# jamesli1618/Obj-GAN

Measured on AMD Instinct MI355X. Metric: G+D train-step images/sec at 256x256, batch 16 per GPU, higher is better.
Workload: dtype fp32 (fp16x2: operands as two fp16 pieces of x * 2^s on the fp16 MFMA); 1 GPU; stage3_256x256_full_GD_step: RNN_ENCODER+G_NET(3 stages)+PatD x3+ShpD x3+ObjSSD+ObjLSD(ROIAlign)+DAMSM+KL+Adam x9+EMA+IS-monitor; per_gpu_batch=16, global_batch=16, parallelism=dp1, fresh_batch_every_step=True

## Files before the change

### include/objgan_hip.h

```cpp
#ifndef OBJGAN_HIP_H
#define OBJGAN_HIP_H

#ifdef __cplusplus
extern "C" {
#endif

int objgan_roi_align_forward(const float* features, const float* rois, float* output,
                             int num_rois, int roi_cols, int channels, int height, int width,
                             int aligned_height, int aligned_width, float spatial_scale,
                             void* stream);
int objgan_roi_align_backward(const float* top_grad, const float* rois, float* bottom_grad,
                              int batch_size, int num_rois, int roi_cols, int channels,
                              int height, int width, int aligned_height, int aligned_width,
                              float spatial_scale, void* stream);

long objgan_roi_align_backward_ws_floats(int batch_size, int num_rois, int channels, int height, int width,
                                         int aligned_height, int aligned_width);
int objgan_roi_align_backward_ordered(const float* top_grad, const float* rois, float* bottom_grad,
                                      int batch_size, int num_rois, int roi_cols, int channels,
                                      int height, int width, int aligned_height, int aligned_width,
                                      float spatial_scale, float* ws, long ws_floats, void* stream);
int objgan_avgpool2s1_forward(const float* in, float* out, long planes, int ih, int iw, void* stream);
int objgan_avgpool2s1_backward(const float* grad_out, float* grad_in, long planes, int ih, int iw,
                               void* stream);

long objgan_conv_packed_floats(int M, int C, int T);
int objgan_conv_bank_layout(int N, int C, int H, int W, int M, int Tg, int PH, int PW, int act, int math);
int objgan_conv_igemm(const float* x, const float* w, const float* bias, float* y, float* wt,
                      int N, int C, int H, int W, int upsample, int pad_mode,
                      int Cout, int Cin, int Torig, int transpose,
                      int Tg, const int* dh, const int* dw, const int* src_tap,
                      int PH, int PW, int stride,
                      int OHf, int OWf, int osh, int osw, int ooh, int oow,
                      int act, int y_prezeroed, int wt_packed, int math, float* ring, const float* xmax, float* ymax,
                      float* ws, long ws_floats, void* stream);
int objgan_absmax_partials(const float* x, long n, float* out1024, void* stream);
long objgan_h2_records_floats(int N, int C, long HW);
int objgan_h2_records(const float* x, const float* xmax1024, void* rec, int N, int C, long HW, void* stream);
long objgan_conv_igemm_ws_floats(int N, int C, int H, int W, int upsample, int pad_mode,
                                 int Cout, int Cin, int Torig, int transpose, int Tg,
                                 int PH, int PW, int stride, int OHf, int OWf, int osh, int osw,
                                 int act, int y_prezeroed, int math, int ring);
int objgan_conv_igemm_plan(int N, int C, int H, int W, int upsample, int pad_mode,
                           int Cout, int Cin, int Torig, int transpose, int Tg,
                           int PH, int PW, int stride, int OHf, int OWf, int osh, int osw,
                           int act, int y_prezeroed, int math, int ring, int* out);
int objgan_reflect_ring_fold(const float* ring, float* y, long planes, int H, int W, void* stream);
long objgan_conv_dgrad_s2_phases_ws_floats(int N, int Cout, int OH, int OW, int math);
int objgan_conv_dgrad_s2_phases_plan(int N, int Cout, int OH, int OW, int Cin, int Tg, int PH, int PW, int math, int* out);
long objgan_conv_dgrad_s2_thin_floats(int Cout, int Cin);
int objgan_conv_pack_job_thin_phase(void* job, const float* w, float* wt, int Cout, int Cin, int phase);
int objgan_conv_dgrad_s2_thin(const float* dy, const float* w, float* dx, float* wt, int N, int Cout, int OH, int OW,
                              int Cin, int wt_packed, void* stream);
int objgan_conv_dgrad_s2_phases(const float* x, const float* w, float* y, float* wt,
                                int N, int Cout, int OH, int OW, int Cin, int Torig,
                                int Tg, const int* dh, const int* dw, const int* src_tap,
                                int PH, int PW, int wt_packed, int math, const float* xmax, float* ws, long ws_floats,
                                void* stream);
long objgan_conv_wgrad_ws_floats(int N, int Cin, int H, int W, int upsample, int pad_mode,
                                 int Cout, int OH, int OW, int ksize, int stride, int pad, int math);
int objgan_conv_wgrad_plan(int N, int Cin, int H, int W, int upsample, int pad_mode,
                           int Cout, int OH, int OW, int ksize, int stride, int pad, int math, int* out);
int objgan_conv_wgrad(const float* x, const float* dy, float* dw,
                      int N, int Cin, int H, int W, int upsample, int pad_mode,
                      int Cout, int OH, int OW, int ksize, int stride, int pad, int math,
                      int accumulate, const float* xmax, const float* dymax, float* ws, long ws_floats, void* stream);
int objgan_conv_wgrad_rec_ok(int N, int Cin, int H, int W, int Cout, int OH, int OW, int ksize);
long objgan_nhwc_bf16_floats(int N, int C, long HW);
int objgan_nhwc_bf16(const float* x, float* out, int N, int C, long HW, void* stream);
int objgan_conv_wgrad_bfb_ok(int N, int Cin, int H, int W, int Cout, int OH, int OW, int ksize);

int objgan_lstm_bidir_forward(const float* table, const long* captions, const int* lens,
                              const float* wt_ih, const float* wt_hh, const float* b_ih, const float* b_hh,
                              float* out, float* hn, int B, int L, int Lout, int I, int H, int ntoken,
                              void* stream);
int objgan_lstm_bidir_forward_state(const float* table, const long* captions, const int* lens,
                                    const float* wt_ih, const float* wt_hh, const float* b_ih, const float* b_hh,
                                    float* out, float* hn, float* cn, int B, int L, int Lout, int I, int H,
                                    int ntoken, void* stream);

int objgan_box_decode_default_cpw(void);
int objgan_box_decode(const float* h0, const float* c0, const double* noise,
                      const float* l_emb, const float* xy_w, const float* xy_b, const float* wh_w, const float* wh_b,
                      const float* nxy_w, const float* nxy_b, const float* wt_ih, const float* wt_hh,
                      const float* b_ih, const float* b_hh, const float* lo_wt, const float* lo_b,
                      const float* xyo_wt, const float* xyo_b, const float* who_wt, const float* who_b,
                      float x0, float y0, float w0, float r0,
                      int* labels, int* lengths, double* samples, float* trace,
                      int B, int T, int H, int L, int K, int A, int sos, int eos, int cpw, void* stream);

long objgan_box_train_ws_floats(int B, int T, int H, int L, int K, int A);
int objgan_box_train_forward(const float* h0, const float* c0, const int* labels, const float* boxes, const int* lens,
                             const float* l_emb, const float* xy_w, const float* xy_b, const float* wh_w,
                             const float* wh_b, const float* nxy_w, const float* nxy_b, const float* wt_ih,
                             const float* wt_hh, const float* b_ih, const float* b_hh, const float* lo_wt,
                             const float* lo_b, const float* xyo_wt, const float* xyo_b, const float* who_wt,
                             const float* who_b, float x0, float y0, float w0, float r0, float* trace, float* ws,
                             long ws_floats, int B, int T, int H, int L, int K, int A, int cpw, void* stream);
int objgan_box_train_loss(const float* trace, const int* labels, const float* boxes, const int* lens,
                          const float* weight, float lamda1, float lamda2, double* sums, float* dtrace,
                          int B, int T, int L, int K, int pad, void* stream);
int objgan_box_train_backward(const float* dtrace, const float* trace, const float* c0, const int* labels,
                              const int* lens, const float* wt_ih, const float* wt_hh, const float* lo_wt,
                              const float* xyo_wt, const float* who_wt, float* const* grads, float* ws, long ws_floats,
                              int B, int T, int H, int L, int K, int A, int cpw, void* stream);
int objgan_box_train_clip(const float* g, long n, float max_norm, double* partials, float* out, void* stream);

long objgan_norm_ws_floats(int N, int C, int HW, int per_channel);
int objgan_norm_forward(const float* x, float* y, const float* residual,
                        const float* gamma, const float* beta,
                        float* running_mean, float* running_var,
                        float* sums, float* mean, float* rstd,
                        int N, int C, int HW, int per_channel, int mode,
                        float eps, float momentum, float* amax, void* stream);
int objgan_norm_amax_supported(int N, int C, int HW, int per_channel, int affine);
int objgan_norm_apply(const float* x, float* y, const float* residual, const float* gamma, const float* beta,
                      const float* mean, const float* rstd, int N, int C, int HW, int per_channel, int mode,
                      void* stream);
int objgan_norm_backward(const float* x, const float* dy, const float* mean, const float* rstd,
                         const float* gamma, const float* beta, float* bsums,
                         float* dx, float* dgamma, float* dbeta,
                         int N, int C, int HW, int per_channel, int mode, float* amax, void* stream);
int objgan_act_backward(const float* dy, const float* y, float* dz, long total, int kind, float* amax, void* stream);
long objgan_channel_sum_ws_floats(int N, int C, int HW);
int objgan_channel_sum(const float* x, float* out, int N, int C, int HW, float* ws, void* stream);

int objgan_attn_general_forward(const float* x, const float* src, const unsigned char* mask,
                                float* wc, float* attn, int B, int idf, int Q, int L, void* stream);
long objgan_attn_general_backward_ws_floats(int B, int idf, int Q, int L);
int objgan_attn_general_backward(const float* x, const float* src, const float* attn,
                                 const float* dwc, const float* dattn, float* dx, float* dsrc,
                                 int B, int idf, int Q, int L, float* ws, void* stream);
int objgan_attn_bu_forward(const float* tgt, const float* ctx1, const float* src,
                           const unsigned char* mask, float* wc, float* attn,
                           int B, int d2, int idf, int R, int L, int normalize, float eps,
                           void* stream);
int objgan_attn_bu_backward(const float* dwc, const float* attn, float* dsrc,
                            int B, int idf, int R, int L, void* stream);
int objgan_masked_max_forward(const float* f, const float* m, float* out, int B, int num, int R,
                              int P, long m_stride_b, long m_stride_r, long m_stride_c, void* stream);
long objgan_masked_max_backward_ws_floats(int B, int num, int R, int P);
int objgan_masked_max_backward(const float* f, const float* m, const float* dout, float* df,
                               int B, int num, int R, int P, long m_stride_b, long m_stride_r,
                               long m_stride_c, float* ws, void* stream);
int objgan_softmax_strided_forward(const float* x, float* y, long outer, int dim, long inner,
                                   float scale, const int* lens, int nlens,
                                   const unsigned char* rowvalid, void* stream);
int objgan_softmax_strided_backward(const float* y, const float* dy, float* dx, long outer, int dim,
                                    long inner, float scale, void* stream);

int objgan_bilinear_forward(const float* x, float* y, long planes, int ih, int iw, int oh, int ow,
                            void* stream);
int objgan_bilinear_backward(const float* dy, float* dx, long planes, int ih, int iw, int oh, int ow,
                             void* stream);
int objgan_sum2x2(const float* dy, float* dx, long planes, int h, int w, void* stream);
int objgan_reflect_fold(const float* dxp, float* dx, long planes, int h, int w, void* stream);
int objgan_bce_const_forward(const float* p, float* out, int n, float t, void* stream);
int objgan_bce_const_backward(const float* p, const float* g, float* dp, int n, float t, void* stream);
int objgan_conv_pack_job_bytes();
int objgan_conv_pack_job(void* job, const float* w, float* wt, int N, int C, int H, int W, int Cout, int Cin,
                         int Torig, int transpose, int Tg, const int* src_tap, int PH, int PW, int act, int math);
int objgan_conv_pack_job_phase(void* job, const float* w, float* wt, int Cout, int Cin, int Torig, int Tg,
                               const int* src_tap_phase, int phase, int math);
int objgan_conv_pack_jobs_run(const void* jobs_dev, int njobs, void* stream);
int objgan_bmm_strided(const float* A, const float* B, float* C, int batch, int M, int N, int K,
                       long sab, long sam, long sak, long sbb, long sbk, long sbn,
                       long scb, long scm, long scn, void* stream);
int objgan_lift_taps_forward(const float* z, const float* bias, float* y, float* scratch, int N, int Mo, int h,
                             int w, int SH, int SW, const int* ci0, const int* ci1, const float* cl1,
                             const int* ri0, const int* ri1, const float* rl1, void* stream);
int objgan_lift_taps_backward(const float* dy, float* dz, float* scratch, int N, int Mo, int h, int w, int SH,
                              int SW, const int* roff, const int* ridx, const float* rwt, const int* coff,
                              const int* cidx, const float* cwt, void* stream);
int objgan_pool2d_forward(const float* x, float* y, int* idx, long planes, int H, int W, int OH, int OW,
                          int k, int s, int p, int mode, void* stream);
int objgan_pool2d_backward(const float* dy, const int* idx, float* dx, long planes, int H, int W, int OH,
                           int OW, int k, int s, int p, int mode, void* stream);
int objgan_adam_step(float* p, const float* g, float* m, float* v, long n, double lr, double beta1,
                     double beta2, double eps, int step, float grad_scale, void* stream);
int objgan_adam_step_gated(float* p, const float* g, float* m, float* v, long n, double lr, double beta1,
                           double beta2, double eps, double* state, const float* flag, float* coef,
                           float grad_scale, void* stream);
int objgan_ema_update(float* avg, const float* p, long n, float decay, float one_minus_decay,
                      void* stream);

int objgan_resize_pil_kmax(int max_in, int S);
int objgan_resize_pil_rgb8(const unsigned char* src, const long* offs, const int* hs, const int* ws, int B,
                           int Hmax, int kmax, int S, int* coef_scratch, unsigned char* tmp_scratch, float* out,
                           void* stream);

long objgan_jpeg_desc_bytes(void);
long objgan_jpeg_seg_bytes(void);
int objgan_jpeg_parse(const unsigned char* file, long nbytes, void* desc_out);
long objgan_jpeg_plan(void* descs, int n, const long* file_offsets, const long* out_offsets, const int* nsegs);
int objgan_jpeg_decode(const unsigned char* files, const void* descs_host, const void* descs_dev, int n,
                       unsigned char* out, void* ws, long ws_bytes, const void* index_in, void* index_out, void* stream);

int objgan_mask_resize(const double* src, int count, int n, int nsizes, const int* sizes, double* const* out,
                       const int* ntaps, const double* taps, void* stream);

int objgan_bilinear_halfpixel_forward(const float* x, float* y, int N, int C, int H, int W, int OH, int OW,
                                      const float* scale, const float* shift, void* stream);
int objgan_moments_accumulate(const float* x, int rows, int D, double* sum, double* outer, void* stream);
int objgan_moments_finalize(const double* sum, const double* outer, long n, int D, double* mu, double* sigma,
                            void* stream);

long objgan_snapshot_ws_doubles(int nvis, int T, int a, int vis);
int objgan_snapshot_blend_table(unsigned char* table65536);
int objgan_snapshot_grid(const float* imgs, const float* lr_imgs, const float* attn, const int* counts, const double* M,
                         const unsigned char* strip, unsigned char* out, double* ws, long ws_doubles,
                         int nvis, int T, int a, int vis, int H, int W, int LH, int LW,
                         int max_word_num, int font_max, int per_panel_norm, void* stream);
int objgan_mask_to_rgb8(const float* masks, const int* sel, unsigned char* out, int N, int HW, void* stream);

int objgan_convlstm_cell_forward(const float* gx, const float* gh, const float* c_prev, float* h_out, float* h_slab,
                                 float* c_out, float* acts, int B, int Ch, int HW, long gx_bstride, long slab_bstride,
                                 void* stream);
int objgan_convlstm_cell_backward(const float* dh_slab, const float* dh_rec, const float* dc_in, const float* acts,
                                  const float* c_prev, float* dg_slab, float* dg_out, float* dc_out, int B, int Ch, int HW,
                                  long dh_bstride, long dg_bstride, void* stream);
int objgan_box_max_forward(const float* x, float* y, unsigned char* arg, int B, int R, long CSS, void* stream);
int objgan_box_max_backward(const float* dy, const unsigned char* arg, float* dx, int B, int R, long CSS, void* stream);
int objgan_boxmaps_onehot(const float* raw, const int* cat, const int* num, float* fwd, float* bwd, int B, int NB, int R,
                          int C, int SS, void* stream);

int objgan_layout_from_decode(const int* labels, const int* lengths, const double* samples, const double* mean_std,
                              const int* label_to_cat, const int* cat_to_rel, const int* thresholds,
                              double* boxes, int* nbox, double* rois, double* fm_rois, int* num_rois, int* cats,
                              float* maps, float* fmaps, int* bounds, const int* sizes, int NB, int F, int R,
                              int min_size, int tie_rule, int B, int T, int L, int ncat, void* stream);

int objgan_pcp_stem_forward(const float* x, float* y, int N, int S, int OH, int OW, void* stream);
int objgan_pcp_stem_backward(const float* dy, float* dx, int N, int S, int OH, int OW, void* stream);
long objgan_l1_tap_ws_doubles(long n);
int objgan_l1_tap_forward(const float* f, const float* r, long n, float* out, int slot, double* ws, void* stream);
int objgan_l1_tap_backward(const float* f, const float* r, const float* gdown, const float* coef, float* g, long n,
                           int relu_mask, float* amax, void* stream);

int objgan_prof_enable(int on);
int objgan_prof_collect(double* ms, double* flops, long* count);
int objgan_prof_dump(float* ms, double* flops, int* meta, int max_records, int* n_out);

#ifdef __cplusplus
}
#endif
#endif
```

### obj-gan_amd/csrc/norm.hip

```cpp
#include "common.h"

#define OG_NORM_NONE 0
#define OG_NORM_LRELU 1
#define OG_NORM_GLU 2

struct NormGeom {
    int N, C, HW;
    int per_channel;
};

__device__ __forceinline__ float og_sigmoid(float v) { return 1.0f / (1.0f + expf(-v)); }

struct NormWs { float* sums; float* part; int P; };
__device__ __forceinline__ void og_store_partial2(const NormWs& ws, int g, int idx, float s1, float s2) {
    if (ws.P == 1) { ws.sums[2 * g] = s1; ws.sums[2 * g + 1] = s2; return; }
    float* slot = ws.part + ((size_t)g * ws.P + idx) * 2;
    slot[0] = s1; slot[1] = s2;
}
__global__ __launch_bounds__(256) void norm_partials_sum_kernel(NormWs ws, int G, float* __restrict__ amax) {
    if (amax && blockIdx.x == 0)
        for (int k = threadIdx.x; k < OG_AMAX_SLOTS; k += 256) amax[k] = 0.f;
    const int g = blockIdx.x * blockDim.x + threadIdx.x;
    if (g >= G) return;
    const float* p = ws.part + (size_t)g * ws.P * 2;
    float a = 0.f, b = 0.f;
    for (int k = 0; k < ws.P; ++k) { a += p[2 * k]; b += p[2 * k + 1]; }
    ws.sums[2 * g] = a; ws.sums[2 * g + 1] = b;
}

__global__ __launch_bounds__(256) void norm_stats_kernel(const float* __restrict__ x,
                                                         NormWs ws, NormGeom gm) {
    __shared__ float red[16];
    const int g = blockIdx.x;
    const int planes = gm.per_channel ? gm.N : 1;
    const size_t base = gm.per_channel ? (size_t)g * gm.HW : (size_t)g * gm.HW;
    const size_t pstride = (size_t)gm.C * gm.HW;
    const long total = (long)planes * gm.HW;
    const float K = x[base];
    const long chunk = (total + gridDim.y - 1) / gridDim.y;
    const long e0 = (long)blockIdx.y * chunk;
    const long e1 = min(total, e0 + chunk);
    float s1 = 0.f, s2 = 0.f;
    for (long e = e0 + threadIdx.x; e < e1; e += blockDim.x) {
        const long p = e / gm.HW;
        const long i = e - p * gm.HW;
        const float d = x[base + p * pstride + i] - K;
        s1 += d;
        s2 += d * d;
    }
    s1 = og_block_sum(s1, red);
    s2 = og_block_sum(s2, red);
    if (threadIdx.x == 0) og_store_partial2(ws, g, blockIdx.y, s1, s2);
}

__global__ __launch_bounds__(256) void norm_finalize_kernel(
    const float* __restrict__ x, const float* __restrict__ sums, float* __restrict__ mean,
    float* __restrict__ rstd, float* __restrict__ running_mean, float* __restrict__ running_var,
    NormGeom gm, int G, float eps, float momentum) {
    const int g = blockIdx.x * blockDim.x + threadIdx.x;
    if (g >= G) return;
    const float cnt = gm.per_channel ? (float)gm.N * gm.HW : (float)gm.HW;
    const float K = x[(size_t)g * gm.HW];
    const float m1 = sums[2 * g] / cnt;
    float var = sums[2 * g + 1] / cnt - m1 * m1;
    var = fmaxf(var, 0.f);
    const float mu = K + m1;
    mean[g] = mu;
    rstd[g] = 1.0f / sqrtf(var + eps);
    if (running_mean) {
        const float unbiased = cnt > 1.f ? var * cnt / (cnt - 1.f) : var;
        running_mean[g] = (1.f - momentum) * running_mean[g] + momentum * mu;
        running_var[g] = (1.f - momentum) * running_var[g] + momentum * unbiased;
    }
}

__global__ __launch_bounds__(256) void norm_apply_kernel(
    const float* __restrict__ x, const float* __restrict__ mean, const float* __restrict__ rstd,
    const float* __restrict__ gamma, const float* __restrict__ beta,
    const float* __restrict__ residual, float* __restrict__ y, NormGeom gm, int mode) {
    const int Co = mode == OG_NORM_GLU ? gm.C / 2 : gm.C;
    const long total = (long)gm.N * Co * gm.HW;
    for (long e = (long)blockIdx.x * blockDim.x + threadIdx.x; e < total;
         e += (long)gridDim.x * blockDim.x) {
        const long plane = e / gm.HW;
        const int i = (int)(e - plane * gm.HW);
        const int n = (int)(plane / Co);
        const int c = (int)(plane - (long)n * Co);
        const int ga = gm.per_channel ? c : n * gm.C + c;
        const size_t xa = ((size_t)n * gm.C + c) * gm.HW + i;
        float za = (x[xa] - mean[ga]) * rstd[ga];
        if (gamma) za = za * gamma[c] + beta[c];
        float v;
        if (mode == OG_NORM_GLU) {
            const int cb = c + Co;
            const int gb = gm.per_channel ? cb : n * gm.C + cb;
            float zb = (x[xa + (size_t)Co * gm.HW] - mean[gb]) * rstd[gb];
            if (gamma) zb = zb * gamma[cb] + beta[cb];
            v = za * og_sigmoid(zb);
        } else if (mode == OG_NORM_LRELU) {
            v = za > 0.f ? za : 0.2f * za;
        } else {
            v = za;
        }
        if (residual) v += residual[e];
        y[e] = v;
    }
}

__device__ __forceinline__ float norm_dz(const float* __restrict__ x, const float* __restrict__ dy,
                                         const float* __restrict__ mean, const float* __restrict__ rstd,
                                         const float* __restrict__ gamma, const float* __restrict__ beta,
                                         const NormGeom& gm, int mode, int n, int c, int i,
                                         float& xhat_out) {
    const int g = gm.per_channel ? c : n * gm.C + c;
    const size_t xa = ((size_t)n * gm.C + c) * gm.HW + i;
    const float xhat = (x[xa] - mean[g]) * rstd[g];
    xhat_out = xhat;
    if (mode == OG_NORM_NONE) return dy[xa];
    float z = xhat;
    if (gamma) z = z * gamma[c] + beta[c];
    if (mode == OG_NORM_LRELU) return dy[xa] * (z > 0.f ? 1.f : 0.2f);
    const int Ch = gm.C / 2;
    const bool is_gate = c >= Ch;
    const int co = is_gate ? c - Ch : c;
    const int cp = is_gate ? c - Ch : c + Ch;
    const int gp = gm.per_channel ? cp : n * gm.C + cp;
    const size_t xp = ((size_t)n * gm.C + cp) * gm.HW + i;
    float zp = (x[xp] - mean[gp]) * rstd[gp];
    if (gamma) zp = zp * gamma[cp] + beta[cp];
    const float d = dy[((size_t)n * Ch + co) * gm.HW + i];
    if (!is_gate) return d * og_sigmoid(zp);
    const float sg = og_sigmoid(z);
    return d * zp * sg * (1.f - sg);
}

__global__ __launch_bounds__(256) void norm_bwd_stats_kernel(
    const float* __restrict__ x, const float* __restrict__ dy, const float* __restrict__ mean,
    const float* __restrict__ rstd, const float* __restrict__ gamma, const float* __restrict__ beta,
    NormWs ws, NormGeom gm, int mode) {
    __shared__ float red[16];
    const int g = blockIdx.x;
    const int planes = gm.per_channel ? gm.N : 1;
    const long total = (long)planes * gm.HW;
    const long chunk = (total + gridDim.y - 1) / gridDim.y;
    const long e0 = (long)blockIdx.y * chunk;
    const long e1 = min(total, e0 + chunk);
    float s1 = 0.f, s2 = 0.f;
    for (long e = e0 + threadIdx.x; e < e1; e += blockDim.x) {
        const int p = (int)(e / gm.HW);
        const int i = (int)(e - (long)p * gm.HW);
        const int n = gm.per_channel ? p : g / gm.C;
        const int c = gm.per_channel ? g : g - n * gm.C;
        float xhat;
        const float dz = norm_dz(x, dy, mean, rstd, gamma, beta, gm, mode, n, c, i, xhat);
        s1 += dz;
        s2 += dz * xhat;
    }
    s1 = og_block_sum(s1, red);
    s2 = og_block_sum(s2, red);
    if (threadIdx.x == 0) og_store_partial2(ws, g, blockIdx.y, s1, s2);
}

__global__ __launch_bounds__(256) void norm_bwd_apply_kernel(
    const float* __restrict__ x, const float* __restrict__ dy, const float* __restrict__ mean,
    const float* __restrict__ rstd, const float* __restrict__ gamma, const float* __restrict__ beta,
    const float* __restrict__ bsums, float* __restrict__ dx, NormGeom gm, int mode) {
    const long total = (long)gm.N * gm.C * gm.HW;
    const float inv_cnt = 1.0f / (gm.per_channel ? (float)gm.N * gm.HW : (float)gm.HW);
    for (long e = (long)blockIdx.x * blockDim.x + threadIdx.x; e < total;
         e += (long)gridDim.x * blockDim.x) {
        const long plane = e / gm.HW;
        const int i = (int)(e - plane * gm.HW);
        const int n = (int)(plane / gm.C);
        const int c = (int)(plane - (long)n * gm.C);
        const int g = gm.per_channel ? c : n * gm.C + c;
        float xhat;
        const float dz = norm_dz(x, dy, mean, rstd, gamma, beta, gm, mode, n, c, i, xhat);
        const float gw = gamma ? gamma[c] : 1.f;
        dx[e] = gw * rstd[g] * (dz - bsums[2 * g] * inv_cnt - xhat * bsums[2 * g + 1] * inv_cnt);
    }
}

#define OG_NORM_CHUNK 8192

__device__ __forceinline__ float og_group_mean(const float* p, int g) { return p[g]; }

__global__ __launch_bounds__(256) void norm_stats_plane_kernel(const float* __restrict__ x,
                                                               NormWs ws, NormGeom gm) {
    __shared__ float red[16];
    const int plane = blockIdx.x;
    const int c = plane % gm.C;
    const int g = gm.per_channel ? c : plane;
    const float K = x[(size_t)g * gm.HW];
    const float4* xp = reinterpret_cast<const float4*>(x + (size_t)plane * gm.HW);
    const int i0 = blockIdx.y * (OG_NORM_CHUNK / 4);
    const int i1 = min(gm.HW / 4, i0 + OG_NORM_CHUNK / 4);
    float s1 = 0.f, s2 = 0.f;
    for (int i = i0 + threadIdx.x; i < i1; i += 256) {
        const float4 v = xp[i];
        const float a = v.x - K, b = v.y - K, cc = v.z - K, d = v.w - K;
        s1 += (a + b) + (cc + d);
        s2 += (a * a + b * b) + (cc * cc + d * d);
    }
    s1 = og_block_sum(s1, red);
    s2 = og_block_sum(s2, red);
    const int idx = gm.per_channel ? (plane / gm.C) * (int)gridDim.y + (int)blockIdx.y : (int)blockIdx.y;
    if (threadIdx.x == 0) og_store_partial2(ws, g, idx, s1, s2);
}

struct NormFin { const float* sums; float* mean_out; float* rstd_out; float* running_mean; float* running_var;
                 float eps, momentum; };

__device__ __forceinline__ void og_group_stats(const float* __restrict__ x, const NormFin& fin, const NormGeom& gm,
                                               int g, bool publish, float& mu, float& rs) {
    const float cnt = gm.per_channel ? (float)gm.N * gm.HW : (float)gm.HW;
    const float K = x[(size_t)g * gm.HW];
    const float m1 = fin.sums[2 * g] / cnt;
    float var = fin.sums[2 * g + 1] / cnt - m1 * m1;
    var = fmaxf(var, 0.f);
    mu = K + m1;
    rs = 1.0f / sqrtf(var + fin.eps);
    if (publish && threadIdx.x == 0) {
        fin.mean_out[g] = mu;
        fin.rstd_out[g] = rs;
        if (fin.running_mean) {
            const float unbiased = cnt > 1.f ? var * cnt / (cnt - 1.f) : var;
            fin.running_mean[g] = (1.f - fin.momentum) * fin.running_mean[g] + fin.momentum * mu;
            fin.running_var[g] = (1.f - fin.momentum) * fin.running_var[g] + fin.momentum * unbiased;
        }
    }
}

template <int MODE>
__global__ __launch_bounds__(256) void norm_apply_plane_kernel(
    const float* __restrict__ x, const float* __restrict__ mean, const float* __restrict__ rstd,
    const float* __restrict__ gamma, const float* __restrict__ beta,
    const float* __restrict__ residual, float* __restrict__ y, NormGeom gm, NormFin fin, float* __restrict__ amax) {
    __shared__ float amax_red[4];
    float vmax = 0.f;
    const int Co = MODE == OG_NORM_GLU ? gm.C / 2 : gm.C;
    const int plane = blockIdx.x;
    const int n = plane / Co;
    const int c = plane - n * Co;
    const int ga = gm.per_channel ? c : n * gm.C + c;
    const bool publish = blockIdx.y == 0 && (!gm.per_channel || n == 0);
    float mua, rsa;
    if (fin.sums) og_group_stats(x, fin, gm, ga, publish, mua, rsa); else { mua = mean[ga]; rsa = rstd[ga]; }
    float sa = rsa, ta = -mua * sa;
    if (gamma) { ta = ta * gamma[c] + beta[c]; sa *= gamma[c]; }
    float sb = 0.f, tb = 0.f;
    if (MODE == OG_NORM_GLU) {
        const int cb = c + Co;
        const int gb = gm.per_channel ? cb : n * gm.C + cb;
        float mub, rsb;
        if (fin.sums) og_group_stats(x, fin, gm, gb, publish, mub, rsb); else { mub = mean[gb]; rsb = rstd[gb]; }
        sb = rsb; tb = -mub * sb;
        if (gamma) { tb = tb * gamma[cb] + beta[cb]; sb *= gamma[cb]; }
    }
    const float4* xa = reinterpret_cast<const float4*>(x + ((size_t)n * gm.C + c) * gm.HW);
    const float4* xb = reinterpret_cast<const float4*>(x + ((size_t)n * gm.C + c + Co) * gm.HW);
    const float4* rp = residual ? reinterpret_cast<const float4*>(residual + (size_t)plane * gm.HW) : nullptr;
    float4* yp = reinterpret_cast<float4*>(y + (size_t)plane * gm.HW);
    const int i0 = blockIdx.y * (OG_NORM_CHUNK / 4);
    const int i1 = min(gm.HW / 4, i0 + OG_NORM_CHUNK / 4);
    for (int i = i0 + threadIdx.x; i < i1; i += 256) {
        const float4 a = xa[i];
        float z[4] = {a.x * sa + ta, a.y * sa + ta, a.z * sa + ta, a.w * sa + ta};
        float v[4];
        if (MODE == OG_NORM_GLU) {
            const float4 b = xb[i];
            const float zb[4] = {b.x * sb + tb, b.y * sb + tb, b.z * sb + tb, b.w * sb + tb};
#pragma unroll
            for (int j = 0; j < 4; ++j) v[j] = z[j] * og_sigmoid(zb[j]);
        } else if (MODE == OG_NORM_LRELU) {
#pragma unroll
            for (int j = 0; j < 4; ++j) v[j] = z[j] > 0.f ? z[j] : 0.2f * z[j];
        } else {
#pragma unroll
            for (int j = 0; j < 4; ++j) v[j] = z[j];
        }
        if (rp) { const float4 r = rp[i]; v[0] += r.x; v[1] += r.y; v[2] += r.z; v[3] += r.w; }
        yp[i] = make_float4(v[0], v[1], v[2], v[3]);
        vmax = fmaxf(fmaxf(vmax, fmaxf(fabsf(v[0]), fabsf(v[1]))), fmaxf(fabsf(v[2]), fabsf(v[3])));
    }
    if (amax) og_amax_atomic(og_block_max(vmax, amax_red), amax, blockIdx.x + blockIdx.y * gridDim.x);
}

template <int MODE>
__device__ __forceinline__ void norm_dz_pair(float xa, float xb, float d, float ma, float ra, float mb, float rb,
                                             float gaa, float baa, float gab, float bab, bool affine,
                                             float& dza, float& xha, float& dzb, float& xhb) {
    xha = (xa - ma) * ra;
    float za = affine ? xha * gaa + baa : xha;
    if (MODE == OG_NORM_NONE) { dza = d; dzb = 0.f; xhb = 0.f; return; }
    if (MODE == OG_NORM_LRELU) { dza = d * (za > 0.f ? 1.f : 0.2f); dzb = 0.f; xhb = 0.f; return; }
    xhb = (xb - mb) * rb;
    const float zb = affine ? xhb * gab + bab : xhb;
    const float sg = og_sigmoid(zb);
    dza = d * sg;
    dzb = d * za * sg * (1.f - sg);
}

template <int MODE>
__global__ __launch_bounds__(256) void norm_bwd_stats_plane_kernel(
    const float* __restrict__ x, const float* __restrict__ dy, const float* __restrict__ mean,
    const float* __restrict__ rstd, const float* __restrict__ gamma, const float* __restrict__ beta,
    NormWs ws, NormGeom gm) {
    __shared__ float red[16];
    const int Co = MODE == OG_NORM_GLU ? gm.C / 2 : gm.C;
    const int plane = blockIdx.x;
    const int n = plane / Co;
    const int c = plane - n * Co;
    const int cb = c + Co;
    const int ga = gm.per_channel ? c : n * gm.C + c;
    const int gb = gm.per_channel ? cb : n * gm.C + cb;
    const bool affine = gamma != nullptr;
    const float ma = mean[ga], ra = rstd[ga];
    const float mb = MODE == OG_NORM_GLU ? mean[gb] : 0.f, rb = MODE == OG_NORM_GLU ? rstd[gb] : 0.f;
    const float gaa = affine ? gamma[c] : 1.f, baa = affine ? beta[c] : 0.f;
    const float gab = (affine && MODE == OG_NORM_GLU) ? gamma[cb] : 1.f, bab = (affine && MODE == OG_NORM_GLU) ? beta[cb] : 0.f;
    const float4* xa = reinterpret_cast<const float4*>(x + ((size_t)n * gm.C + c) * gm.HW);
    const float4* xb = reinterpret_cast<const float4*>(x + ((size_t)n * gm.C + cb) * gm.HW);
    const float4* dp = reinterpret_cast<const float4*>(dy + (size_t)plane * gm.HW);
    const int i0 = blockIdx.y * (OG_NORM_CHUNK / 4);
    const int i1 = min(gm.HW / 4, i0 + OG_NORM_CHUNK / 4);
    float a1 = 0.f, a2 = 0.f, b1 = 0.f, b2 = 0.f;
    for (int i = i0 + threadIdx.x; i < i1; i += 256) {
        const float4 va = xa[i];
        const float4 vb = MODE == OG_NORM_GLU ? xb[i] : make_float4(0.f, 0.f, 0.f, 0.f);
        const float4 vd = dp[i];
        const float xs[4] = {va.x, va.y, va.z, va.w}, ys[4] = {vb.x, vb.y, vb.z, vb.w}, ds[4] = {vd.x, vd.y, vd.z, vd.w};
#pragma unroll
        for (int j = 0; j < 4; ++j) {
            float dza, xha, dzb, xhb;
            norm_dz_pair<MODE>(xs[j], ys[j], ds[j], ma, ra, mb, rb, gaa, baa, gab, bab, affine, dza, xha, dzb, xhb);
            a1 += dza; a2 += dza * xha;
            if (MODE == OG_NORM_GLU) { b1 += dzb; b2 += dzb * xhb; }
        }
    }
    a1 = og_block_sum(a1, red);
    a2 = og_block_sum(a2, red);
    if (MODE == OG_NORM_GLU) { b1 = og_block_sum(b1, red); b2 = og_block_sum(b2, red); }
    const int idx = gm.per_channel ? n * (int)gridDim.y + (int)blockIdx.y : (int)blockIdx.y;
    if (threadIdx.x == 0) {
        og_store_partial2(ws, ga, idx, a1, a2);
        if (MODE == OG_NORM_GLU) og_store_partial2(ws, gb, idx, b1, b2);
    }
}

template <int MODE>
__global__ __launch_bounds__(256) void norm_bwd_apply_plane_kernel(
    const float* __restrict__ x, const float* __restrict__ dy, const float* __restrict__ mean,
    const float* __restrict__ rstd, const float* __restrict__ gamma, const float* __restrict__ beta,
    const float* __restrict__ bsums, float* __restrict__ dx, NormGeom gm,
    float* __restrict__ dgamma, float* __restrict__ dbeta, float* __restrict__ amax) {
    __shared__ float amax_red[4];
    float vmax = 0.f;
    const int Co = MODE == OG_NORM_GLU ? gm.C / 2 : gm.C;
    const int plane = blockIdx.x;
    const int n = plane / Co;
    const int c = plane - n * Co;
    const int cb = c + Co;
    const int ga = gm.per_channel ? c : n * gm.C + c;
    const int gb = gm.per_channel ? cb : n * gm.C + cb;
    const bool affine = gamma != nullptr;
    const float inv_cnt = 1.0f / (gm.per_channel ? (float)gm.N * gm.HW : (float)gm.HW);
    if (dgamma && gm.per_channel && n == 0 && blockIdx.y == 0 && threadIdx.x == 0) {
        dbeta[c] = bsums[2 * c]; dgamma[c] = bsums[2 * c + 1];
        if (MODE == OG_NORM_GLU) { dbeta[cb] = bsums[2 * cb]; dgamma[cb] = bsums[2 * cb + 1]; }
    }
    const float ma = mean[ga], ra = rstd[ga];
    const float mb = MODE == OG_NORM_GLU ? mean[gb] : 0.f, rb = MODE == OG_NORM_GLU ? rstd[gb] : 0.f;
    const float gaa = affine ? gamma[c] : 1.f, baa = affine ? beta[c] : 0.f;
    const float gab = (affine && MODE == OG_NORM_GLU) ? gamma[cb] : 1.f, bab = (affine && MODE == OG_NORM_GLU) ? beta[cb] : 0.f;
    const float ka1 = bsums[2 * ga] * inv_cnt, ka2 = bsums[2 * ga + 1] * inv_cnt;
    const float kb1 = MODE == OG_NORM_GLU ? bsums[2 * gb] * inv_cnt : 0.f, kb2 = MODE == OG_NORM_GLU ? bsums[2 * gb + 1] * inv_cnt : 0.f;
    const float wa = gaa * ra, wb = gab * rb;
    const float4* xa = reinterpret_cast<const float4*>(x + ((size_t)n * gm.C + c) * gm.HW);
    const float4* xb = reinterpret_cast<const float4*>(x + ((size_t)n * gm.C + cb) * gm.HW);
    const float4* dp = reinterpret_cast<const float4*>(dy + (size_t)plane * gm.HW);
    float4* oa = reinterpret_cast<float4*>(dx + ((size_t)n * gm.C + c) * gm.HW);
    float4* ob = reinterpret_cast<float4*>(dx + ((size_t)n * gm.C + cb) * gm.HW);
    const int i0 = blockIdx.y * (OG_NORM_CHUNK / 4);
    const int i1 = min(gm.HW / 4, i0 + OG_NORM_CHUNK / 4);
    for (int i = i0 + threadIdx.x; i < i1; i += 256) {
        const float4 va = xa[i];
        const float4 vb = MODE == OG_NORM_GLU ? xb[i] : make_float4(0.f, 0.f, 0.f, 0.f);
        const float4 vd = dp[i];
        const float xs[4] = {va.x, va.y, va.z, va.w}, ys[4] = {vb.x, vb.y, vb.z, vb.w}, ds[4] = {vd.x, vd.y, vd.z, vd.w};
        float ra4[4], rb4[4];
#pragma unroll
        for (int j = 0; j < 4; ++j) {
            float dza, xha, dzb, xhb;
            norm_dz_pair<MODE>(xs[j], ys[j], ds[j], ma, ra, mb, rb, gaa, baa, gab, bab, affine, dza, xha, dzb, xhb);
            ra4[j] = wa * (dza - ka1 - xha * ka2);
            rb4[j] = wb * (dzb - kb1 - xhb * kb2);
        }
        oa[i] = make_float4(ra4[0], ra4[1], ra4[2], ra4[3]);
        if (MODE == OG_NORM_GLU) ob[i] = make_float4(rb4[0], rb4[1], rb4[2], rb4[3]);
#pragma unroll
        for (int j = 0; j < 4; ++j) vmax = fmaxf(vmax, fmaxf(fabsf(ra4[j]), MODE == OG_NORM_GLU ? fabsf(rb4[j]) : 0.f));
    }
    if (amax) og_amax_atomic(og_block_max(vmax, amax_red), amax, blockIdx.x + blockIdx.y * gridDim.x);
}


__device__ __forceinline__ void og_block_sum2(float& a, float& b, float* red) {
    a = og_wave_sum(a);
    b = og_wave_sum(b);
    const int lane = threadIdx.x & 63, wid = threadIdx.x >> 6;
    __syncthreads();
    if (lane == 0) { red[wid] = a; red[4 + wid] = b; }
    __syncthreads();
    a = red[0] + red[1] + red[2] + red[3];
    b = red[4] + red[5] + red[6] + red[7];
}

template <int MODE>
__global__ __launch_bounds__(256) void in_fwd_fused_kernel(
    const float* __restrict__ x, const float* __restrict__ residual, float* __restrict__ y,
    float* __restrict__ mean, float* __restrict__ rstd, NormGeom gm, float eps, float* __restrict__ amax) {
    __shared__ float red[8];
    float vmax = 0.f;
    const int Co = MODE == OG_NORM_GLU ? gm.C / 2 : gm.C;
    const int plane = blockIdx.x;
    const int n = plane / Co;
    const int c = plane - n * Co;
    const int ga = n * gm.C + c, gb = ga + Co;
    const float4* xa = reinterpret_cast<const float4*>(x + (size_t)ga * gm.HW);
    const float4* xb = reinterpret_cast<const float4*>(x + (size_t)gb * gm.HW);
    const int n4 = gm.HW / 4;
    const float inv = 1.0f / (float)gm.HW;
    const float Ka = x[(size_t)ga * gm.HW];
    float s1 = 0.f, s2 = 0.f;
    for (int i = threadIdx.x; i < n4; i += 256) {
        const float4 v = xa[i];
        const float a = v.x - Ka, b = v.y - Ka, cc = v.z - Ka, d = v.w - Ka;
        s1 += (a + b) + (cc + d);
        s2 += (a * a + b * b) + (cc * cc + d * d);
    }
    og_block_sum2(s1, s2, red);
    float m1 = s1 * inv;
    float var = fmaxf(s2 * inv - m1 * m1, 0.f);
    const float mua = Ka + m1, ra = 1.0f / sqrtf(var + eps);
    float mub = 0.f, rb = 0.f;
    if (MODE == OG_NORM_GLU) {
        const float Kb = x[(size_t)gb * gm.HW];
        s1 = 0.f; s2 = 0.f;
        for (int i = threadIdx.x; i < n4; i += 256) {
            const float4 v = xb[i];
            const float a = v.x - Kb, b = v.y - Kb, cc = v.z - Kb, d = v.w - Kb;
            s1 += (a + b) + (cc + d);
            s2 += (a * a + b * b) + (cc * cc + d * d);
        }
        og_block_sum2(s1, s2, red);
        m1 = s1 * inv;
        var = fmaxf(s2 * inv - m1 * m1, 0.f);
        mub = Kb + m1; rb = 1.0f / sqrtf(var + eps);
    }
    if (threadIdx.x == 0) {
        mean[ga] = mua; rstd[ga] = ra;
        if (MODE == OG_NORM_GLU) { mean[gb] = mub; rstd[gb] = rb; }
    }
    const float sa = ra, ta = -mua * ra, sb = rb, tb = -mub * rb;
    const float4* rp = residual ? reinterpret_cast<const float4*>(residual + (size_t)plane * gm.HW) : nullptr;
    float4* yp = reinterpret_cast<float4*>(y + (size_t)plane * gm.HW);
    for (int i = threadIdx.x; i < n4; i += 256) {
        const float4 a = xa[i];
        const float z[4] = {a.x * sa + ta, a.y * sa + ta, a.z * sa + ta, a.w * sa + ta};
        float v[4];
        if (MODE == OG_NORM_GLU) {
            const float4 b = xb[i];
            const float zb[4] = {b.x * sb + tb, b.y * sb + tb, b.z * sb + tb, b.w * sb + tb};
#pragma unroll
            for (int j = 0; j < 4; ++j) v[j] = z[j] * og_sigmoid(zb[j]);
        } else if (MODE == OG_NORM_LRELU) {
#pragma unroll
            for (int j = 0; j < 4; ++j) v[j] = z[j] > 0.f ? z[j] : 0.2f * z[j];
        } else {
#pragma unroll
            for (int j = 0; j < 4; ++j) v[j] = z[j];
        }
        if (rp) { const float4 r = rp[i]; v[0] += r.x; v[1] += r.y; v[2] += r.z; v[3] += r.w; }
        yp[i] = make_float4(v[0], v[1], v[2], v[3]);
        vmax = fmaxf(fmaxf(vmax, fmaxf(fabsf(v[0]), fabsf(v[1]))), fmaxf(fabsf(v[2]), fabsf(v[3])));
    }
    if (amax) og_amax_atomic(og_block_max(vmax, red), amax, blockIdx.x);
}

template <int MODE>
__global__ __launch_bounds__(256) void in_bwd_fused_kernel(
    const float* __restrict__ x, const float* __restrict__ dy, const float* __restrict__ mean,
    const float* __restrict__ rstd, float* __restrict__ dx, NormGeom gm, float* __restrict__ amax) {
    __shared__ float red[8];
    float vmax = 0.f;
    const int Co = MODE == OG_NORM_GLU ? gm.C / 2 : gm.C;
    const int plane = blockIdx.x;
    const int n = plane / Co;
    const int c = plane - n * Co;
    const int ga = n * gm.C + c, gb = ga + Co;
    const float inv_cnt = 1.0f / (float)gm.HW;
    const float ma = mean[ga], ra = rstd[ga];
    const float mb = MODE == OG_NORM_GLU ? mean[gb] : 0.f, rb = MODE == OG_NORM_GLU ? rstd[gb] : 0.f;
    const float4* xa = reinterpret_cast<const float4*>(x + (size_t)ga * gm.HW);
    const float4* xb = reinterpret_cast<const float4*>(x + (size_t)gb * gm.HW);
    const float4* dp = reinterpret_cast<const float4*>(dy + (size_t)plane * gm.HW);
    float4* oa = reinterpret_cast<float4*>(dx + (size_t)ga * gm.HW);
    float4* ob = reinterpret_cast<float4*>(dx + (size_t)gb * gm.HW);
    const int n4 = gm.HW / 4;
    float a1 = 0.f, a2 = 0.f, b1 = 0.f, b2 = 0.f;
    for (int i = threadIdx.x; i < n4; i += 256) {
        const float4 va = xa[i];
        const float4 vb = MODE == OG_NORM_GLU ? xb[i] : make_float4(0.f, 0.f, 0.f, 0.f);
        const float4 vd = dp[i];
        const float xs[4] = {va.x, va.y, va.z, va.w}, ys[4] = {vb.x, vb.y, vb.z, vb.w}, ds[4] = {vd.x, vd.y, vd.z, vd.w};
#pragma unroll
        for (int j = 0; j < 4; ++j) {
            float dza, xha, dzb, xhb;
            norm_dz_pair<MODE>(xs[j], ys[j], ds[j], ma, ra, mb, rb, 1.f, 0.f, 1.f, 0.f, false, dza, xha, dzb, xhb);
            a1 += dza; a2 += dza * xha;
            if (MODE == OG_NORM_GLU) { b1 += dzb; b2 += dzb * xhb; }
        }
    }
    og_block_sum2(a1, a2, red);
    if (MODE == OG_NORM_GLU) og_block_sum2(b1, b2, red);
    const float ka1 = a1 * inv_cnt, ka2 = a2 * inv_cnt, kb1 = b1 * inv_cnt, kb2 = b2 * inv_cnt;
    for (int i = threadIdx.x; i < n4; i += 256) {
        const float4 va = xa[i];
        const float4 vb = MODE == OG_NORM_GLU ? xb[i] : make_float4(0.f, 0.f, 0.f, 0.f);
        const float4 vd = dp[i];
        const float xs[4] = {va.x, va.y, va.z, va.w}, ys[4] = {vb.x, vb.y, vb.z, vb.w}, ds[4] = {vd.x, vd.y, vd.z, vd.w};
        float ra4[4], rb4[4];
#pragma unroll
        for (int j = 0; j < 4; ++j) {
            float dza, xha, dzb, xhb;
            norm_dz_pair<MODE>(xs[j], ys[j], ds[j], ma, ra, mb, rb, 1.f, 0.f, 1.f, 0.f, false, dza, xha, dzb, xhb);
            ra4[j] = ra * (dza - ka1 - xha * ka2);
            rb4[j] = rb * (dzb - kb1 - xhb * kb2);
        }
        oa[i] = make_float4(ra4[0], ra4[1], ra4[2], ra4[3]);
        if (MODE == OG_NORM_GLU) ob[i] = make_float4(rb4[0], rb4[1], rb4[2], rb4[3]);
#pragma unroll
        for (int j = 0; j < 4; ++j) vmax = fmaxf(vmax, fmaxf(fabsf(ra4[j]), MODE == OG_NORM_GLU ? fabsf(rb4[j]) : 0.f));
    }
    if (amax) og_amax_atomic(og_block_max(vmax, red), amax, blockIdx.x);
}

__global__ void norm_affine_grad_kernel(const float* __restrict__ bsums, float* __restrict__ dgamma,
                                        float* __restrict__ dbeta, int C) {
    const int c = blockIdx.x * blockDim.x + threadIdx.x;
    if (c < C) { dbeta[c] = bsums[2 * c]; dgamma[c] = bsums[2 * c + 1]; }
}

__device__ __forceinline__ float act_bwd_one(float d, float o, int kind) {
    float r;
    if (kind == 1) r = d * (o > 0.f ? 1.f : 0.2f);
    else if (kind == 2) r = d * (1.f - o * o);
    else if (kind == 3) r = d * o * (1.f - o);
    else r = o > 0.f ? d : 0.f;
    return r;
}
template <bool V4>
__global__ __launch_bounds__(256) void act_bwd_kernel(const float* __restrict__ dy,
                                                      const float* __restrict__ y,
                                                      float* __restrict__ dz, long total, int kind,
                                                      float* __restrict__ amax) {
    __shared__ float amax_red[4];
    float vmax = 0.f;
    long e0 = 0;
    if (V4) {
        const long n4 = total >> 2, step = (long)gridDim.x * 256;
        const float4* d4 = reinterpret_cast<const float4*>(dy);
        const float4* y4 = reinterpret_cast<const float4*>(y);
        float4* z4 = reinterpret_cast<float4*>(dz);
        for (long g = (long)blockIdx.x * 256 + threadIdx.x; g < n4; g += 2 * step) {
            const long g1 = g + step < n4 ? g + step : g;
            const float4 da = d4[g], oa = y4[g], db = d4[g1], ob = y4[g1];
            const float ra[4] = {act_bwd_one(da.x, oa.x, kind), act_bwd_one(da.y, oa.y, kind),
                                 act_bwd_one(da.z, oa.z, kind), act_bwd_one(da.w, oa.w, kind)};
            const float rb[4] = {act_bwd_one(db.x, ob.x, kind), act_bwd_one(db.y, ob.y, kind),
                                 act_bwd_one(db.z, ob.z, kind), act_bwd_one(db.w, ob.w, kind)};
            z4[g] = make_float4(ra[0], ra[1], ra[2], ra[3]);
            if (g1 != g) z4[g1] = make_float4(rb[0], rb[1], rb[2], rb[3]);
#pragma unroll
            for (int j = 0; j < 4; ++j) vmax = fmaxf(vmax, fmaxf(fabsf(ra[j]), fabsf(rb[j])));
        }
        e0 = n4 << 2;
    }
    for (long e = e0 + (long)blockIdx.x * blockDim.x + threadIdx.x; e < total;
         e += (long)gridDim.x * blockDim.x) {
        const float r = act_bwd_one(dy[e], y[e], kind);
        dz[e] = r;
        vmax = fmaxf(vmax, fabsf(r));
    }
    if (amax) og_amax_own(og_block_max(vmax, amax_red), amax, blockIdx.x, gridDim.x);
}

__global__ __launch_bounds__(256) void channel_sum_kernel(const float* __restrict__ x,
                                                          float* __restrict__ out, int N, int C, int HW,
                                                          float* __restrict__ part) {
    __shared__ float red[16];
    const int c = blockIdx.x;
    const long total = (long)N * HW;
    const long chunk = (total + gridDim.y - 1) / gridDim.y;
    const long e0 = (long)blockIdx.y * chunk;
    const long e1 = min(total, e0 + chunk);
    float s = 0.f;
    for (long e = e0 + threadIdx.x; e < e1; e += blockDim.x) {
        const long n = e / HW;
        const long i = e - n * HW;
        s += x[((size_t)n * C + c) * HW + i];
    }
    s = og_block_sum(s, red);
    if (threadIdx.x == 0) {
        if (gridDim.y == 1) out[c] = s; else part[(size_t)c * gridDim.y + blockIdx.y] = s;
    }
}
__global__ __launch_bounds__(256) void channel_partials_sum_kernel(const float* __restrict__ part, float* __restrict__ out,
                                                                   int C, int S) {
    const int c = blockIdx.x * blockDim.x + threadIdx.x;
    if (c >= C) return;
    float a = 0.f;
    for (int k = 0; k < S; ++k) a += part[(size_t)c * S + k];
    out[c] = a;
}

#define OG_IN_FUSED_MAX 65536
OG_KNOB(og_norm_nofuse, "OG_NORM_NOFUSE", 0)

static inline int norm_splits(int G, long per_group) {
    long want = (256L * 4 + G - 1) / G;
    long maxs = (per_group + 1023) / 1024;
    if (want > maxs) want = maxs;
    if (want < 1) want = 1;
    if (want > 1024) want = 1024;
    return (int)want;
}

static inline bool norm_planes(int N, int C, int HW) { return (HW % 4 == 0) && HW >= 256 && (long)N * C < 2000000; }
static inline int norm_partials(int N, int C, int HW, int per_channel) {
    const int G = per_channel ? C : N * C;
    if (norm_planes(N, C, HW)) return (per_channel ? N : 1) * og_cdiv(HW, OG_NORM_CHUNK);
    return norm_splits(G, per_channel ? (long)N * HW : HW);
}
static inline NormWs norm_ws(float* buf, int G, int P) { return NormWs{buf, buf + 2 * (size_t)G, P}; }
static inline void norm_sum_partials(const NormWs& ws, int G, hipStream_t s, float* amax = nullptr) {
    if (ws.P > 1) hipLaunchKernelGGL(norm_partials_sum_kernel, dim3(og_cdiv(G, 256)), dim3(256), 0, s, ws, G, amax);
}

extern "C" {

int objgan_norm_amax_supported(int N, int C, int HW, int per_channel, int affine) {
    if (N <= 0 || C <= 0 || HW <= 0 || !norm_planes(N, C, HW)) return 0;
    if (!per_channel && !affine && HW <= OG_IN_FUSED_MAX && !og_norm_nofuse()) return 2;
    return norm_partials(N, C, HW, per_channel) > 1 ? 1 : 0;
}

long objgan_norm_ws_floats(int N, int C, int HW, int per_channel) {
    if (N <= 0 || C <= 0 || HW <= 0) return 0;
    const long G = per_channel ? C : (long)N * C;
    return 2 * G + 2 * G * norm_partials(N, C, HW, per_channel);
}

int objgan_norm_forward(const float* x, float* y, const float* residual,
                        const float* gamma, const float* beta,
                        float* running_mean, float* running_var,
                        float* sums, float* mean, float* rstd,
                        int N, int C, int HW, int per_channel, int mode,
                        float eps, float momentum, float* amax, void* stream) {
    OG_ENTRY();
    if (mode == OG_NORM_GLU && (C & 1)) return OG_BAD_ARGS;
    if (N <= 0 || C <= 0 || HW <= 0) return OG_OK;
    if (amax && !objgan_norm_amax_supported(N, C, HW, per_channel, gamma != nullptr)) return OG_BAD_ARGS;
    hipStream_t s = (hipStream_t)stream;
    NormGeom gm{N, C, HW, per_channel};
    const int G = per_channel ? C : N * C;
    const long per_group = per_channel ? (long)N * HW : HW;
    const bool planes = norm_planes(N, C, HW);
    const int chunks = og_cdiv(HW, OG_NORM_CHUNK);
    const int Co = mode == OG_NORM_GLU ? C / 2 : C;
    if (planes && !per_channel && !gamma && HW <= OG_IN_FUSED_MAX && !og_norm_nofuse()) {
        dim3 grid(N * Co);
        if (mode == OG_NORM_GLU)
            hipLaunchKernelGGL((in_fwd_fused_kernel<OG_NORM_GLU>), grid, dim3(256), 0, s, x, residual, y, mean, rstd, gm, eps, amax);
        else if (mode == OG_NORM_LRELU)
            hipLaunchKernelGGL((in_fwd_fused_kernel<OG_NORM_LRELU>), grid, dim3(256), 0, s, x, residual, y, mean, rstd, gm, eps, amax);
        else
            hipLaunchKernelGGL((in_fwd_fused_kernel<OG_NORM_NONE>), grid, dim3(256), 0, s, x, residual, y, mean, rstd, gm, eps, amax);
        return og_launch_status();
    }
    const NormWs ws = norm_ws(sums, G, norm_partials(N, C, HW, per_channel));
    if (planes) {
        hipLaunchKernelGGL(norm_stats_plane_kernel, dim3(N * C, chunks), dim3(256), 0, s, x, ws, gm);
    } else {
        dim3 grid(G, norm_splits(G, per_group));
        hipLaunchKernelGGL(norm_stats_kernel, grid, dim3(256), 0, s, x, ws, gm);
    }
    norm_sum_partials(ws, G, s, amax);
    if (planes) {
        dim3 grid(N * Co, chunks);
        const NormFin fin{sums, mean, rstd, running_mean, running_var, eps, momentum};
        if (mode == OG_NORM_GLU)
            hipLaunchKernelGGL((norm_apply_plane_kernel<OG_NORM_GLU>), grid, dim3(256), 0, s, x, mean, rstd, gamma, beta, residual, y, gm, fin, amax);
        else if (mode == OG_NORM_LRELU)
            hipLaunchKernelGGL((norm_apply_plane_kernel<OG_NORM_LRELU>), grid, dim3(256), 0, s, x, mean, rstd, gamma, beta, residual, y, gm, fin, amax);
        else
            hipLaunchKernelGGL((norm_apply_plane_kernel<OG_NORM_NONE>), grid, dim3(256), 0, s, x, mean, rstd, gamma, beta, residual, y, gm, fin, amax);
        return og_launch_status();
    }
    hipLaunchKernelGGL(norm_finalize_kernel, dim3(og_cdiv(G, 256)), dim3(256), 0, s, x, sums, mean,
                       rstd, running_mean, running_var, gm, G, eps, momentum);
    const long total = (long)N * Co * HW;
    hipLaunchKernelGGL(norm_apply_kernel, dim3(og_stream_grid(total, 256)), dim3(256), 0, s, x, mean,
                       rstd, gamma, beta, residual, y, gm, mode);
    return og_launch_status();
}

int objgan_norm_apply(const float* x, float* y, const float* residual, const float* gamma, const float* beta,
                      const float* mean, const float* rstd, int N, int C, int HW, int per_channel, int mode,
                      void* stream) {
    OG_ENTRY();
    if (mode == OG_NORM_GLU && (C & 1)) return OG_BAD_ARGS;
    if (N <= 0 || C <= 0 || HW <= 0) return OG_OK;
    hipStream_t s = (hipStream_t)stream;
    NormGeom gm{N, C, HW, per_channel};
    const int Co = mode == OG_NORM_GLU ? C / 2 : C;
    if ((HW % 4 == 0) && HW >= 256 && (long)N * C < 2000000) {
        dim3 grid(N * Co, og_cdiv(HW, OG_NORM_CHUNK));
        const NormFin fin{nullptr, nullptr, nullptr, nullptr, nullptr, 0.f, 0.f};
        if (mode == OG_NORM_GLU)
            hipLaunchKernelGGL((norm_apply_plane_kernel<OG_NORM_GLU>), grid, dim3(256), 0, s, x, mean, rstd, gamma, beta, residual, y, gm, fin, (float*)nullptr);
        else if (mode == OG_NORM_LRELU)
            hipLaunchKernelGGL((norm_apply_plane_kernel<OG_NORM_LRELU>), grid, dim3(256), 0, s, x, mean, rstd, gamma, beta, residual, y, gm, fin, (float*)nullptr);
        else
            hipLaunchKernelGGL((norm_apply_plane_kernel<OG_NORM_NONE>), grid, dim3(256), 0, s, x, mean, rstd, gamma, beta, residual, y, gm, fin, (float*)nullptr);
        return og_launch_status();
    }
    const long total = (long)N * Co * HW;
    hipLaunchKernelGGL(norm_apply_kernel, dim3(og_stream_grid(total, 256)), dim3(256), 0, s, x, mean,
                       rstd, gamma, beta, residual, y, gm, mode);
    return og_launch_status();
}

int objgan_norm_backward(const float* x, const float* dy, const float* mean, const float* rstd,
                         const float* gamma, const float* beta, float* bsums,
                         float* dx, float* dgamma, float* dbeta,
                         int N, int C, int HW, int per_channel, int mode, float* amax, void* stream) {
    OG_ENTRY();
    if (mode == OG_NORM_GLU && (C & 1)) return OG_BAD_ARGS;
    if (N <= 0 || C <= 0 || HW <= 0) return OG_OK;
    if (amax && !objgan_norm_amax_supported(N, C, HW, per_channel, gamma != nullptr)) return OG_BAD_ARGS;
    hipStream_t s = (hipStream_t)stream;
    NormGeom gm{N, C, HW, per_channel};
    const int G = per_channel ? C : N * C;
    const long per_group = per_channel ? (long)N * HW : HW;
    const bool planes = norm_planes(N, C, HW);
    if (planes && !per_channel && !gamma && HW <= OG_IN_FUSED_MAX && !og_norm_nofuse()) {
        const int Co = mode == OG_NORM_GLU ? C / 2 : C;
        dim3 grid(N * Co);
        if (mode == OG_NORM_GLU)
            hipLaunchKernelGGL((in_bwd_fused_kernel<OG_NORM_GLU>), grid, dim3(256), 0, s, x, dy, mean, rstd, dx, gm, amax);
        else if (mode == OG_NORM_LRELU)
            hipLaunchKernelGGL((in_bwd_fused_kernel<OG_NORM_LRELU>), grid, dim3(256), 0, s, x, dy, mean, rstd, dx, gm, amax);
        else
            hipLaunchKernelGGL((in_bwd_fused_kernel<OG_NORM_NONE>), grid, dim3(256), 0, s, x, dy, mean, rstd, dx, gm, amax);
        return og_launch_status();
    }
    const NormWs ws = norm_ws(bsums, G, norm_partials(N, C, HW, per_channel));
    if (planes) {
        const int Co = mode == OG_NORM_GLU ? C / 2 : C;
        dim3 grid(N * Co, og_cdiv(HW, OG_NORM_CHUNK));
#define OG_NB(MODE)                                                                                         \
        hipLaunchKernelGGL((norm_bwd_stats_plane_kernel<MODE>), grid, dim3(256), 0, s, x, dy, mean, rstd,   \
                           gamma, beta, ws, gm);                                                            \
        norm_sum_partials(ws, G, s, amax);                                                                  \
        hipLaunchKernelGGL((norm_bwd_apply_plane_kernel<MODE>), grid, dim3(256), 0, s, x, dy, mean, rstd,   \
                           gamma, beta, bsums, dx, gm, dgamma, dbeta, amax);
        if (mode == OG_NORM_GLU) { OG_NB(OG_NORM_GLU) } else if (mode == OG_NORM_LRELU) { OG_NB(OG_NORM_LRELU) } else { OG_NB(OG_NORM_NONE) }
#undef OG_NB
        return og_launch_status();
    } else {
        dim3 grid(G, norm_splits(G, per_group));
        hipLaunchKernelGGL(norm_bwd_stats_kernel, grid, dim3(256), 0, s, x, dy, mean, rstd, gamma, beta,
                           ws, gm, mode);
        norm_sum_partials(ws, G, s);
        const long total = (long)N * C * HW;
        hipLaunchKernelGGL(norm_bwd_apply_kernel, dim3(og_stream_grid(total, 256)), dim3(256), 0, s, x,
                           dy, mean, rstd, gamma, beta, bsums, dx, gm, mode);
    }
    if (dgamma && per_channel)
        hipLaunchKernelGGL(norm_affine_grad_kernel, dim3(og_cdiv(C, 256)), dim3(256), 0, s, bsums,
                           dgamma, dbeta, C);
    return og_launch_status();
}

int objgan_act_backward(const float* dy, const float* y, float* dz, long total, int kind, float* amax,
                        void* stream) {
    OG_ENTRY();
    if (kind < 1 || kind > 4) return OG_BAD_ARGS;
    if (total <= 0) return OG_OK;
    const bool v4 = !(((size_t)dy | (size_t)y | (size_t)dz) & 15) && total >= 4;
    int grid = og_stream_grid(v4 ? (total + 3) >> 2 : total, 256);
    if (amax && grid > OG_AMAX_SLOTS) grid = OG_AMAX_SLOTS;
    if (v4) hipLaunchKernelGGL(act_bwd_kernel<true>, dim3(grid), dim3(256), 0, (hipStream_t)stream, dy, y, dz, total, kind, amax);
    else hipLaunchKernelGGL(act_bwd_kernel<false>, dim3(grid), dim3(256), 0, (hipStream_t)stream, dy, y, dz, total, kind, amax);
    return og_launch_status();
}

long objgan_channel_sum_ws_floats(int N, int C, int HW) {
    if (N <= 0 || C <= 0 || HW <= 0) return 0;
    const int S = norm_splits(C, (long)N * HW);
    return S > 1 ? (long)C * S : 0;
}

int objgan_channel_sum(const float* x, float* out, int N, int C, int HW, float* ws, void* stream) {
    OG_ENTRY();
    if (N <= 0 || C <= 0 || HW <= 0) return OG_OK;
    hipStream_t s = (hipStream_t)stream;
    const int S = norm_splits(C, (long)N * HW);
    if (S > 1 && !ws) return OG_BAD_ARGS;
    dim3 grid(C, S);
    hipLaunchKernelGGL(channel_sum_kernel, grid, dim3(256), 0, s, x, out, N, C, HW, ws);
    if (S > 1) hipLaunchKernelGGL(channel_partials_sum_kernel, dim3(og_cdiv(C, 256)), dim3(256), 0, s, ws, out, C, S);
    return og_launch_status();
}

}
```

### obj-gan_amd/objgan_hip/_lib.py

```python
import ctypes
import os

from . import build as _build

_c_int = ctypes.c_int
_c_long = ctypes.c_long
_c_float = ctypes.c_float
_c_double = ctypes.c_double
_ptr = ctypes.c_void_p

SIGNATURES = {
    "objgan_roi_align_forward": [_ptr, _ptr, _ptr, _c_int, _c_int, _c_int, _c_int, _c_int, _c_int, _c_int, _c_float, _ptr],
    "objgan_roi_align_backward": [_ptr, _ptr, _ptr, _c_int, _c_int, _c_int, _c_int, _c_int, _c_int, _c_int, _c_int, _c_float, _ptr],
    "objgan_roi_align_backward_ordered": [_ptr, _ptr, _ptr, _c_int, _c_int, _c_int, _c_int, _c_int, _c_int, _c_int, _c_int,
                                          _c_float, _ptr, _c_long, _ptr],
    "objgan_avgpool2s1_forward": [_ptr, _ptr, _c_long, _c_int, _c_int, _ptr],
    "objgan_avgpool2s1_backward": [_ptr, _ptr, _c_long, _c_int, _c_int, _ptr],
    "objgan_conv_igemm": [_ptr, _ptr, _ptr, _ptr, _ptr,
                          _c_int, _c_int, _c_int, _c_int, _c_int, _c_int,
                          _c_int, _c_int, _c_int, _c_int,
                          _c_int, _ptr, _ptr, _ptr,
                          _c_int, _c_int, _c_int,
                          _c_int, _c_int, _c_int, _c_int, _c_int, _c_int,
                          _c_int, _c_int, _c_int, _c_int, _ptr, _ptr, _ptr, _ptr, _c_long, _ptr],
    "objgan_absmax_partials": [_ptr, _c_long, _ptr, _ptr],
    "objgan_h2_records": [_ptr, _ptr, _ptr, _c_int, _c_int, _c_long, _ptr],
    "objgan_reflect_ring_fold": [_ptr, _ptr, _c_long, _c_int, _c_int, _ptr],
    "objgan_conv_dgrad_s2_phases": [_ptr, _ptr, _ptr, _ptr, _c_int, _c_int, _c_int, _c_int, _c_int, _c_int,
                                    _c_int, _ptr, _ptr, _ptr, _c_int, _c_int, _c_int, _c_int, _ptr, _ptr, _c_long, _ptr],
    "objgan_conv_wgrad": [_ptr, _ptr, _ptr, _c_int, _c_int, _c_int, _c_int, _c_int, _c_int,
                          _c_int, _c_int, _c_int, _c_int, _c_int, _c_int, _c_int, _c_int, _ptr, _ptr, _ptr, _c_long, _ptr],
    "objgan_lstm_bidir_forward": [_ptr, _ptr, _ptr, _ptr, _ptr, _ptr, _ptr, _ptr, _ptr,
                                  _c_int, _c_int, _c_int, _c_int, _c_int, _c_int, _ptr],
    "objgan_lstm_bidir_forward_state": [_ptr] * 10 + [_c_int] * 6 + [_ptr],
    "objgan_box_decode_default_cpw": [],
    "objgan_box_decode": [_ptr] * 20 + [_c_float] * 4 + [_ptr] * 4 + [_c_int] * 9 + [_ptr],
    "objgan_box_train_forward": [_ptr] * 22 + [_c_float] * 4 + [_ptr, _ptr, _c_long] + [_c_int] * 7 + [_ptr],
    "objgan_box_train_loss": [_ptr] * 5 + [_c_float] * 2 + [_ptr, _ptr] + [_c_int] * 5 + [_ptr],
    "objgan_box_train_backward": [_ptr] * 12 + [_c_long] + [_c_int] * 7 + [_ptr],
    "objgan_box_train_clip": [_ptr, _c_long, _c_float, _ptr, _ptr, _ptr],
    "objgan_norm_forward": [_ptr, _ptr, _ptr, _ptr, _ptr, _ptr, _ptr, _ptr, _ptr, _ptr,
                            _c_int, _c_int, _c_int, _c_int, _c_int, _c_float, _c_float, _ptr, _ptr],
    "objgan_norm_amax_supported": [_c_int] * 5,
    "objgan_norm_apply": [_ptr, _ptr, _ptr, _ptr, _ptr, _ptr, _ptr, _c_int, _c_int, _c_int, _c_int, _c_int, _ptr],
    "objgan_norm_backward": [_ptr, _ptr, _ptr, _ptr, _ptr, _ptr, _ptr, _ptr, _ptr, _ptr,
                             _c_int, _c_int, _c_int, _c_int, _c_int, _ptr, _ptr],
    "objgan_act_backward": [_ptr, _ptr, _ptr, _c_long, _c_int, _ptr, _ptr],
    "objgan_channel_sum": [_ptr, _ptr, _c_int, _c_int, _c_int, _ptr, _ptr],
    "objgan_attn_general_forward": [_ptr, _ptr, _ptr, _ptr, _ptr, _c_int, _c_int, _c_int, _c_int, _ptr],
    "objgan_attn_general_backward": [_ptr, _ptr, _ptr, _ptr, _ptr, _ptr, _ptr, _c_int, _c_int, _c_int, _c_int, _ptr, _ptr],
    "objgan_attn_bu_forward": [_ptr, _ptr, _ptr, _ptr, _ptr, _ptr, _c_int, _c_int, _c_int, _c_int, _c_int, _c_int, _c_float, _ptr],
    "objgan_attn_bu_backward": [_ptr, _ptr, _ptr, _c_int, _c_int, _c_int, _c_int, _ptr],
    "objgan_masked_max_forward": [_ptr, _ptr, _ptr, _c_int, _c_int, _c_int, _c_int, _c_long, _c_long, _c_long, _ptr],
    "objgan_masked_max_backward": [_ptr, _ptr, _ptr, _ptr, _c_int, _c_int, _c_int, _c_int, _c_long, _c_long, _c_long, _ptr, _ptr],
    "objgan_softmax_strided_forward": [_ptr, _ptr, _c_long, _c_int, _c_long, _c_float, _ptr, _c_int, _ptr, _ptr],
    "objgan_softmax_strided_backward": [_ptr, _ptr, _ptr, _c_long, _c_int, _c_long, _c_float, _ptr],
    "objgan_bilinear_forward": [_ptr, _ptr, _c_long, _c_int, _c_int, _c_int, _c_int, _ptr],
    "objgan_bilinear_backward": [_ptr, _ptr, _c_long, _c_int, _c_int, _c_int, _c_int, _ptr],
    "objgan_bilinear_halfpixel_forward": [_ptr, _ptr, _c_int, _c_int, _c_int, _c_int, _c_int, _c_int, _ptr, _ptr, _ptr],
    "objgan_moments_accumulate": [_ptr, _c_int, _c_int, _ptr, _ptr, _ptr],
    "objgan_moments_finalize": [_ptr, _ptr, _c_long, _c_int, _ptr, _ptr, _ptr],
    "objgan_sum2x2": [_ptr, _ptr, _c_long, _c_int, _c_int, _ptr],
    "objgan_reflect_fold": [_ptr, _ptr, _c_long, _c_int, _c_int, _ptr],
    "objgan_conv_pack_job_bytes": [],
    "objgan_conv_pack_job": [_ptr, _ptr, _ptr, _c_int, _c_int, _c_int, _c_int, _c_int, _c_int, _c_int, _c_int,
                             _c_int, _ptr, _c_int, _c_int, _c_int, _c_int],
    "objgan_conv_pack_job_phase": [_ptr, _ptr, _ptr, _c_int, _c_int, _c_int, _c_int, _ptr, _c_int, _c_int],
    "objgan_conv_pack_job_thin_phase": [_ptr, _ptr, _ptr, _c_int, _c_int, _c_int],
    "objgan_conv_dgrad_s2_thin": [_ptr, _ptr, _ptr, _ptr, _c_int, _c_int, _c_int, _c_int, _c_int, _c_int, _ptr],
    "objgan_conv_pack_jobs_run": [_ptr, _c_int, _ptr],
    "objgan_bce_const_forward": [_ptr, _ptr, _c_int, _c_float, _ptr],
    "objgan_bce_const_backward": [_ptr, _ptr, _ptr, _c_int, _c_float, _ptr],
    "objgan_bmm_strided": [_ptr, _ptr, _ptr, _c_int, _c_int, _c_int, _c_int] + [_c_long] * 9 + [_ptr],
    "objgan_lift_taps_forward": [_ptr, _ptr, _ptr, _ptr, _c_int, _c_int, _c_int, _c_int, _c_int, _c_int,
                                 _ptr, _ptr, _ptr, _ptr, _ptr, _ptr, _ptr],
    "objgan_lift_taps_backward": [_ptr, _ptr, _ptr, _c_int, _c_int, _c_int, _c_int, _c_int, _c_int,
                                  _ptr, _ptr, _ptr, _ptr, _ptr, _ptr, _ptr],
    "objgan_pool2d_forward": [_ptr, _ptr, _ptr, _c_long, _c_int, _c_int, _c_int, _c_int, _c_int, _c_int, _c_int, _c_int, _ptr],
    "objgan_pool2d_backward": [_ptr, _ptr, _ptr, _c_long, _c_int, _c_int, _c_int, _c_int, _c_int, _c_int, _c_int, _c_int, _ptr],
    "objgan_adam_step": [_ptr, _ptr, _ptr, _ptr, _c_long, _c_double, _c_double, _c_double, _c_double, _c_int, _c_float, _ptr],
    "objgan_adam_step_gated": [_ptr, _ptr, _ptr, _ptr, _c_long, _c_double, _c_double, _c_double, _c_double,
                               _ptr, _ptr, _ptr, _c_float, _ptr],
    "objgan_ema_update": [_ptr, _ptr, _c_long, _c_float, _c_float, _ptr],
    "objgan_resize_pil_kmax": [_c_int, _c_int],
    "objgan_resize_pil_rgb8": [_ptr, _ptr, _ptr, _ptr, _c_int, _c_int, _c_int, _c_int, _ptr, _ptr, _ptr, _ptr],
    "objgan_mask_resize": [_ptr, _c_int, _c_int, _c_int, _ptr, _ptr, _ptr, _ptr, _ptr],
    "objgan_jpeg_parse": [ctypes.c_char_p, _c_long, _ptr],
    "objgan_jpeg_decode": [_ptr, _ptr, _ptr, _c_int, _ptr, _ptr, _c_long, _ptr, _ptr, _ptr],
    "objgan_snapshot_blend_table": [_ptr],
    "objgan_snapshot_grid": [_ptr, _ptr, _ptr, _ptr, _ptr, _ptr, _ptr, _ptr, _c_long] + [_c_int] * 11 + [_ptr],
    "objgan_mask_to_rgb8": [_ptr, _ptr, _ptr, _c_int, _c_int, _ptr],
    "objgan_convlstm_cell_forward": [_ptr] * 7 + [_c_int] * 3 + [_c_long] * 2 + [_ptr],
    "objgan_convlstm_cell_backward": [_ptr] * 8 + [_c_int] * 3 + [_c_long] * 2 + [_ptr],
    "objgan_box_max_forward": [_ptr, _ptr, _ptr, _c_int, _c_int, _c_long, _ptr],
    "objgan_box_max_backward": [_ptr, _ptr, _ptr, _c_int, _c_int, _c_long, _ptr],
    "objgan_boxmaps_onehot": [_ptr] * 5 + [_c_int] * 5 + [_ptr],
    "objgan_layout_from_decode": [_ptr] * 17 + [_c_int] * 9 + [_ptr],
    "objgan_pcp_stem_forward": [_ptr, _ptr, _c_int, _c_int, _c_int, _c_int, _ptr],
    "objgan_pcp_stem_backward": [_ptr, _ptr, _c_int, _c_int, _c_int, _c_int, _ptr],
    "objgan_l1_tap_forward": [_ptr, _ptr, _c_long, _ptr, _c_int, _ptr, _ptr],
    "objgan_l1_tap_backward": [_ptr, _ptr, _ptr, _ptr, _ptr, _c_long, _c_int, _ptr, _ptr],
    "objgan_prof_enable": [_c_int],
    "objgan_conv_bank_layout": [_c_int] * 10,
    "objgan_conv_wgrad_rec_ok": [_c_int] * 8,
    "objgan_conv_wgrad_bfb_ok": [_c_int] * 8,
    "objgan_conv_igemm_plan": [_c_int] * 22 + [_ptr],
    "objgan_conv_dgrad_s2_phases_plan": [_c_int] * 9 + [_ptr],
    "objgan_conv_wgrad_plan": [_c_int] * 13 + [_ptr],
    "objgan_nhwc_bf16": [_ptr, _ptr, _c_int, _c_int, _c_long, _ptr],
    "objgan_prof_collect": [_ptr, _ptr, _ptr],
    "objgan_prof_dump": [_ptr, _ptr, _ptr, _c_int, _ptr],
}
LONG_RETURN = {"objgan_conv_packed_floats": [_c_int, _c_int, _c_int],
               "objgan_conv_igemm_ws_floats": [_c_int] * 22,
               "objgan_conv_wgrad_ws_floats": [_c_int] * 13,
               "objgan_conv_dgrad_s2_phases_ws_floats": [_c_int] * 5,
               "objgan_conv_dgrad_s2_thin_floats": [_c_int, _c_int],
               "objgan_h2_records_floats": [_c_int, _c_int, _c_long],
               "objgan_nhwc_bf16_floats": [_c_int, _c_int, _c_long],
               "objgan_norm_ws_floats": [_c_int] * 4,
               "objgan_box_train_ws_floats": [_c_int] * 6,
               "objgan_attn_general_backward_ws_floats": [_c_int] * 4,
               "objgan_masked_max_backward_ws_floats": [_c_int] * 4,
               "objgan_channel_sum_ws_floats": [_c_int] * 3,
               "objgan_l1_tap_ws_doubles": [_c_long],
               "objgan_roi_align_backward_ws_floats": [_c_int] * 7,
               "objgan_snapshot_ws_doubles": [_c_int] * 4,
               "objgan_jpeg_desc_bytes": [],
               "objgan_jpeg_seg_bytes": [],
               "objgan_jpeg_plan": [_ptr, _c_int, _ptr, _ptr, _ptr]}

_LIB = None


class ObjganHipError(RuntimeError):
    pass


def lib_path():
    return _build.LIB_PATH


def load(build_if_missing=True):
    global _LIB
    if _LIB is not None:
        return _LIB
    path = lib_path()
    if not os.path.exists(path):
        if not build_if_missing:
            raise ObjganHipError("libobjgan_hip.so not built: run `python -c 'import __graft_entry__ as g; g.build()'`")
        _build.build(verbose=False)
    import torch
    lib = ctypes.CDLL(path)
    for name, argtypes in SIGNATURES.items():
        fn = getattr(lib, name)
        fn.argtypes = argtypes
        fn.restype = _c_int
    for name, argtypes in LONG_RETURN.items():
        fn = getattr(lib, name)
        fn.argtypes = argtypes
        fn.restype = _c_long
    _LIB = lib
    return lib


def call(name, *args):
    rc = getattr(load(), name)(*args)
    if rc == 1:
        return
    if rc == 0:
        raise ObjganHipError("%s: invalid arguments (returned 0)" % name)
    raise ObjganHipError("%s: HIP launch failed (hipError %d)" % (name, -rc))
```

### obj-gan_amd/objgan_hip/ops.py

```python
import ctypes
import math

import os

import torch

from . import _lib

_F32 = torch.float32


def _p(t):
    return None if t is None else ctypes.c_void_p(t.data_ptr())


def _stream():
    return ctypes.c_void_p(torch._C._cuda_getCurrentRawStream(torch._C._cuda_getDevice()))


def _chk(*tensors):
    for t in tensors:
        if t is None:
            continue
        if not t.is_cuda:
# ... 401 lines not shown
    if math == 4 and (layout & 255) != 5:
        math = 2
        layout = _q("objgan_conv_bank_layout", N, C, H, W, M, Tg, PH, PW, act, math)
    xmax = _absmax(x) if math == 4 else None
    if math == 4 and _H2_CENSUS is not None:
        _census("data gradient: filter columns (input channels)" if transpose else "forward: filter rows (output channels)",
                w, 1 if transpose else 0, site)
    kmath, xk = math, x
    if math == 1 and _B16["on"] and _BF16_CHANNELS_LAST and (layout & 255) == 3:
        xc = _bf16_copy(x, N, C, H * W)
        if xc is not None:
            kmath, xk = 3, xc
    if math == 4 and _REC["on"] and not (x.data_ptr() & 15):
        rec = _records(x, xmax, N, C, H * W, 2.0 * M * Tg * PH * PW / float(H * W), M)
        if rec is not None:
            kmath, xk = 5, rec

    def pack_jobs(wt):
        job = _job_blob()
        _lib.call("objgan_conv_pack_job", job, _p(w), _p(wt), N, C, H, W, Cout, Cin, Torig, int(transpose),
                  Tg, _iarr(src_tap), PH, PW, act, math)
        return [job.raw]

    key = _pack_key(w, transpose, src_tap, layout, math) if cache else None
    wt, packed = _bank_acquire(key, w, _q("objgan_conv_packed_floats", int(M), int(C), int(Tg)), x.device, pack_jobs, "igemm")
    nws = _q("objgan_conv_igemm_ws_floats", N, C, H, W, int(upsample), int(pad_mode), Cout, Cin, Torig,
                                                   int(transpose), Tg, PH, PW, stride, OHf, OWf, osh, osw, act,
                                                   int(y_prezeroed), kmath, 0 if ring is None else 1)
    ws = torch.empty(nws, dtype=_F32, device=x.device) if nws > 0 else None
    if not _BF16_CHANNELS_LAST and math == 1 and nws == _nhwc_floats(N, C, H, W):
        ws, nws = None, 0
    _lib.call("objgan_conv_igemm", _p(xk), _p(w), _p(bias), _p(y), _p(wt),
              N, C, H, W, int(upsample), int(pad_mode), Cout, Cin, Torig, int(transpose),
              Tg, _iarr(dh), _iarr(dw), _iarr(src_tap), PH, PW, stride,
              OHf, OWf, osh, osw, ooh, oow, act, int(y_prezeroed), packed, kmath, _p(ring), _p(xmax), _p(ymax),
              _p(ws), nws, _stream())


def _dgrad_s2_phases(g, w, N, Cout, OH, OW, Cin, k, pad_h, pad_w, LH, LW, cacheable=True):
    KH, KW = (k, k) if isinstance(k, int) else k
    if KH % 2 or KW % 2 or LH % 2 or LW % 2 or Cin <= 32:
        return None
    if float(N) * Cout * OH * OW * 4.0 >= 4.0e9:
        return None
    dh, dw, st = [], [], []
    for a in range(2):
        for b in range(2):
            th, tw, ts = _taps(KH, KW, a + pad_h, b + pad_w, 2)
            dh, dw, st = dh + th, dw + tw, st + ts
    Tg = len(st) // 4
    if Tg > 8:
        return None
    dx = torch.empty((N, Cin, LH, LW), dtype=_F32, device=g.device)
    n = 4 * ((Cin * Tg * ((Cout + 15) // 16 * 16) * 3 + 1) // 2) + _AMAX_SLOTS
    math = _call_math(2.0 * Cin * Cout * Tg * N * LH * LW)
    site = ("conv", w.data_ptr(), 1)
    if math == 4 and _demoted(site):
        math = 2
    xmax = _absmax(g) if math == 4 else None
    if math == 4 and _H2_CENSUS is not None:
        _census("data gradient: filter columns (input channels)", w, 1, site)

    def pack_jobs(wt):
        jobs = []
        for ph in range(4):
            job = _job_blob()
            _lib.call("objgan_conv_pack_job_phase", job, _p(w), _p(wt), Cout, Cin, KH * KW, Tg,
                      _iarr(st[ph * Tg:(ph + 1) * Tg]), ph, math)
            jobs.append(job.raw)
        return jobs

    wt, packed = _bank_acquire(_pack_key(w, 2, st, False, math) if cacheable else None, w, n, g.device, pack_jobs, "phases")
    nws = _q("objgan_conv_dgrad_s2_phases_ws_floats", N, Cout, OH, OW, math)
    ws = torch.empty(nws, dtype=_F32, device=g.device) if nws > 0 and _BF16_CHANNELS_LAST else None
    nws = nws if ws is not None else 0
    kmath, gk = math, g
    if math == 4 and _REC["on"] and not (g.data_ptr() & 15):
        rec = _records(g, xmax, N, Cout, OH * OW, 2.0 * Cin * Tg * LH * LW / float(OH * OW), Cin)
        if rec is not None:
            kmath, gk = 5, rec
    _lib.call("objgan_conv_dgrad_s2_phases", _p(gk), _p(w), _p(dx), _p(wt), N, Cout, OH, OW, Cin, KH * KW,
              Tg, _iarr(dh), _iarr(dw), _iarr(st), LH // 2, LW // 2, packed, kmath, _p(xmax), _p(ws), nws, _stream())
    return dx


_THIN4 = {"on": _os.environ.get("OBJGAN_THIN4", "1") != "0"}


def _dgrad_s2_thin(g, w, N, Cout, OH, OW, Cin, cacheable=True):
    dx = torch.empty((N, Cin, 2 * OH, 2 * OW), dtype=_F32, device=g.device)
    n = _q("objgan_conv_dgrad_s2_thin_floats", Cout, Cin)

    def pack_jobs(wt):
        jobs = []
        for ph in range(4):
            job = _job_blob()
            _lib.call("objgan_conv_pack_job_thin_phase", job, _p(w), _p(wt), Cout, Cin, ph)
            jobs.append(job.raw)
        return jobs

    wt, packed = _bank_acquire(_pack_key(w, 3, (0,), "thin4", 0) if cacheable else None, w, n, g.device, pack_jobs, "thin4")
    _lib.call("objgan_conv_dgrad_s2_thin", _p(g), _p(w), _p(dx), _p(wt), N, Cout, OH, OW, Cin, packed, _stream())
    return dx


def conv_out_size(L, k, s, p):
    return (L + 2 * p - k) // s + 1


def _pair(v):
    return (v, v) if isinstance(v, int) else v


def _taps(KH, KW, oh, ow, step=1, sign=1):
    khs = [kh for kh in range(KH) if (oh - kh) % step == 0]
    kws = [kw for kw in range(KW) if (ow - kw) % step == 0]
    return ([sign * ((oh - kh) // step) for kh in khs for kw in kws],
            [sign * ((ow - kw) // step) for kh in khs for kw in kws],
            [kh * KW + kw for kh in khs for kw in kws])


def _conv_fwd(x, w, bias, stride, pad, refl, upsample, act):
    N, Cin, H, W = x.shape
    Cout, Cin2, KH, KW = w.shape
    if Cin2 != Cin or KH * KW > 32:
        raise _lib.ObjganHipError("convolution: unsupported filter %s for input %s" % (tuple(w.shape), tuple(x.shape)))
    ph, pw = _pair(pad)
    LH, LW = (2 * H, 2 * W) if upsample else (H, W)
    OH, OW = conv_out_size(LH, KH, stride, ph), conv_out_size(LW, KW, stride, pw)
    y = torch.empty((N, Cout, OH, OW), dtype=_F32, device=x.device)
    dh, dw, st = _taps(KH, KW, ph, pw, sign=-1)
    ym = _amax_zeroed(x.device) if (act in ("lrelu", "relu") and _amax_wanted(y.numel())) else None
    _igemm(x, w, bias, y, N, Cin, H, W, upsample, refl, Cout, Cin, KH * KW, 0,
           dh, dw, st, OH, OW, stride, OH, OW, 1, 1, 0, 0, _ACT[act], ymax=ym)
    if ym is not None:
        _amax_attach(y, ym)
    return y


def _conv_dgrad(g, w, N, Cin, H, W, stride, pad, refl, upsample, cacheable=True):
    Cout, KH, KW = w.shape[0], w.shape[2], w.shape[3]
    T = KH * KW
    ph, pw = _pair(pad)
    OH, OW = g.shape[2], g.shape[3]
    LH, LW = (2 * H, 2 * W) if upsample else (H, W)
    if stride == 1:
        TH, TW = (LH + 2 * ph, LW + 2 * pw) if refl else (LH, LW)
        dh, dw, st = _taps(KH, KW, 0, 0) if refl else _taps(KH, KW, ph, pw)
        ring_ok = (refl and (ph, pw) == (1, 1) and LH >= 3 and LW >= 3 and
                   (_q("objgan_conv_bank_layout", N, Cout, OH, OW, Cin, T, TH, TW, 0, _MATH["mode"]) & 255) in (1, 3, 4, 5))
        if ring_ok:
            dxl = torch.empty((N, Cin, LH, LW), dtype=_F32, device=g.device)
            ring = torch.empty((N * Cin, 2 * TW + 2 * TH), dtype=_F32, device=g.device)
            _igemm(g, w, None, dxl, N, Cout, OH, OW, 0, 0, Cout, Cin, T, 1,
                   dh, dw, st, TH, TW, 1, LH, LW, 1, 1, 0, 0, 0, ring=ring, cache=cacheable)
            _lib.call("objgan_reflect_ring_fold", _p(ring), _p(dxl), N * Cin, LH, LW, _stream())
        else:
            dxl = torch.empty((N, Cin, TH, TW), dtype=_F32, device=g.device)
            _igemm(g, w, None, dxl, N, Cout, OH, OW, 0, 0, Cout, Cin, T, 1,
                   dh, dw, st, TH, TW, 1, TH, TW, 1, 1, 0, 0, 0, cache=cacheable)
            if refl:
                folded = torch.empty((N, Cin, LH, LW), dtype=_F32, device=g.device)
                _lib.call("objgan_reflect_fold", _p(dxl), _p(folded), N * Cin, LH, LW, _stream())
                dxl = folded
    elif stride == 2:
        if refl:
            raise _lib.ObjganHipError("stride-2 reflect conv is not on the hot path")
        dxl = None
        if (_THIN4["on"] and (KH, KW) == (4, 4) and (ph, pw) == (1, 1) and Cin <= 12 and LH == 2 * OH and LW == 2 * OW
                and N * OH * OW >= 65536 and float(N) * Cout * OH * OW * 4.0 < 4.0e9):
            dxl = _dgrad_s2_thin(g, w, N, Cout, OH, OW, Cin, cacheable)
        if dxl is None:
            dxl = _dgrad_s2_phases(g, w, N, Cout, OH, OW, Cin, (KH, KW), ph, pw, LH, LW, cacheable)
        phases = range(2) if dxl is None else ()
        if dxl is None:
            dxl = torch.zeros((N, Cin, LH, LW), dtype=_F32, device=g.device)
        for a in phases:
            PHg = (LH - a + 1) // 2
            for b in range(2):
                PWg = (LW - b + 1) // 2
                if PHg <= 0 or PWg <= 0:
                    continue
                dh, dw, st = _taps(KH, KW, a + ph, b + pw, 2)
                if not st:
                    dh, dw, st = [0], [0], [-1]
                _igemm(g, w, None, dxl, N, Cout, OH, OW, 0, 0, Cout, Cin, T, 1,
                       dh, dw, st, PHg, PWg, 1, LH, LW, 2, 2, a, b, 0, y_prezeroed=1, cache=cacheable)
    else:
        raise _lib.ObjganHipError("conv2d backward: stride %d not supported" % stride)
    if upsample:
        dx = torch.empty((N, Cin, H, W), dtype=_F32, device=g.device)
        _lib.call("objgan_sum2x2", _p(dxl), _p(dx), N * Cin, H, W, _stream())
        return dx
    return dxl


_WG_ASYNC = {"stream": None, "pending": []}


class wgrad_stream_scope(object):
    def __init__(self, stream):
        self.stream = stream

    def __enter__(self):
        self.prev = _WG_ASYNC["stream"]
        _WG_ASYNC["stream"] = self.stream
        return self

    def __exit__(self, *exc):
        _WG_ASYNC["stream"] = self.prev
        return False


def wgrad_join():
    if _WG_ASYNC["pending"]:
        cur = torch.cuda.current_stream()
        for st in _WG_ASYNC["pending"]:
            cur.wait_stream(st)
        del _WG_ASYNC["pending"][:]


def _conv_wgrad(x, g, Cout, k, stride, pad, refl, upsample, sink=None):
    N, Cin, H, W = x.shape
    if sink is not None:
        dw_ = sink[0]
    else:
        dw_ = torch.empty((Cout, Cin, k, k), dtype=_F32, device=x.device)
    math = _call_math(2.0 * Cout * Cin * k * k * N * g.shape[2] * g.shape[3])
    site = ("wgrad", sink[0].data_ptr() if sink is not None else 0, N, Cin, H, W, Cout, k, stride, int(upsample), refl)
    if math == 4 and _demoted(site):
        math = 2
    geo = (N, Cin, H, W, int(upsample), refl, Cout, g.shape[2], g.shape[3], k, stride, pad, math)
    xmax, gmax = (_absmax(x), _absmax(g)) if math == 4 else (None, None)
    if math == 4 and _H2_CENSUS is not None:
        _census("weight gradient: x channels (filter columns)", x, 1, site)
        _census("weight gradient: dy channels (filter rows)", g, 1, site)
    xk = x
    rec_pays = bool(upsample) or (refl and H * W <= 4096) or _REC["wgrad"] == "all"
    if (math == 4 and _REC["on"] and _REC["wgrad"] and rec_pays and not (x.data_ptr() & 15) and
            _q("objgan_conv_wgrad_rec_ok", N, Cin, H, W, Cout, g.shape[2], g.shape[3], k)):
        rec = _records(x, xmax, N, Cin, H * W, 2.0 * Cout * k * k * g.shape[2] * g.shape[3] / float(H * W), Cout)
        if rec is not None:
            geo = geo[:-1] + (_REC["wgrad_math"],)
            xk = rec
    if (math == 1 and _B16["on"] and _BF16_CHANNELS_LAST
            and _q("objgan_conv_wgrad_bfb_ok", N, Cin, H, W, Cout, g.shape[2], g.shape[3], k)):
        xc = _bf16_copy(x, N, Cin, H * W)
        if xc is not None:
            geo = geo[:-1] + (3,)
            xk = xc
    nws = _q("objgan_conv_wgrad_ws_floats", *geo)
    side = _WG_ASYNC["stream"] if (sink is not None and _H2_CENSUS is None) else None
    if side is not None:
        cur = torch.cuda.current_stream()
        side.wait_stream(cur)
        for t in (xk, g, xmax, gmax):
            if t is not None:
                t.record_stream(side)
        with torch.cuda.stream(side):
            ws = torch.empty(nws, dtype=_F32, device=x.device) if nws > 0 else None
            _lib.call("objgan_conv_wgrad", _p(xk), _p(g), _p(dw_), *geo, 1, _p(xmax), _p(gmax), _p(ws), nws, _stream())
        if side not in _WG_ASYNC["pending"]:
            _WG_ASYNC["pending"].append(side)
        sink[1]()
        return None
    ws = torch.empty(nws, dtype=_F32, device=x.device) if nws > 0 else None
    _lib.call("objgan_conv_wgrad", _p(xk), _p(g), _p(dw_), *geo, 0 if sink is None else 1, _p(xmax), _p(gmax), _p(ws), nws,
              _stream())
    if sink is not None:
        sink[1]()
        return None
    return dw_


_DIRECT_WGRAD = {"on": False}


def direct_wgrad(on):
    _DIRECT_WGRAD["on"] = bool(on)


class direct_wgrad_scope(object):

    def __init__(self, on=True):
        self.on = bool(on)

    def __enter__(self):
        self.prev = _DIRECT_WGRAD["on"]
        _DIRECT_WGRAD["on"] = self.on
        return self

    def __exit__(self, *exc):
        _DIRECT_WGRAD["on"] = self.prev
        return False


def _grad_sink(w, shape):
    sink = getattr(w, "_og_grad_sink", None) if _DIRECT_WGRAD["on"] else None
    if sink is None or w.grad is None or w.grad.data_ptr() != sink[0].data_ptr() or tuple(sink[0].shape) != tuple(shape):
        return None
    return sink


def _channel_sum(g, out, N, C, HW):
    n = _lib.load().objgan_channel_sum_ws_floats(N, C, HW)
    ws = torch.empty(n, dtype=_F32, device=g.device) if n > 0 else None
    _lib.call("objgan_channel_sum", _p(g), _p(out), N, C, HW, _p(ws), _stream())


def _act_grad(dy, y, act):
    if act in (None, "none"):
        return dy
    g = torch.empty_like(dy)
    am = torch.empty(_AMAX_SLOTS, dtype=_F32, device=dy.device) if _amax_wanted(dy.numel()) else None
    _lib.call("objgan_act_backward", _p(dy), _p(y), _p(g), dy.numel(), _ACT[act], _p(am), _stream())
    if am is not None:
        _amax_attach(g, am)
    return g


class _Conv2dFn(torch.autograd.Function):

    @staticmethod
    def forward(ctx, x, w, bias, stride, pad, pad_mode, upsample, act):
        _chk(x, w, bias)
        x = _c(x)
        w = _c(w)
        if w.shape[1] != x.shape[1] or w.shape[2] != w.shape[3]:
            raise _lib.ObjganHipError("conv2d: bad weight shape %s for input %s" % (tuple(w.shape), tuple(x.shape)))
        refl = 1 if pad_mode == "reflect" else 0
        if refl and pad != 1:
            raise _lib.ObjganHipError("reflect padding is implemented for pad=1")
        y = _conv_fwd(x, w, bias, stride, pad, refl, upsample, act)
        ctx.cfg = (stride, pad, refl, bool(upsample), act, w.shape[2])
        ctx.has_bias = bias is not None
        ctx.save_for_backward(x, w, y if act not in (None, "none") else None)
        return y

    @staticmethod
    def backward(ctx, dy):
        x, w, y = ctx.saved_tensors
        stride, pad, refl, upsample, act, k = ctx.cfg
        N, Cin, H, W = x.shape
        Cout = w.shape[0]
        dy = _c(dy)
        _chk(dy)
        g = _act_grad(dy, y, act)
        dx = dw_ = db = None
        if ctx.needs_input_grad[1]:
            dw_ = _conv_wgrad(x, g, Cout, k, stride, pad, refl, upsample, sink=_grad_sink(w, (Cout, Cin, k, k)))
        if ctx.needs_input_grad[0]:
            dx = _conv_dgrad(g, w, N, Cin, H, W, stride, pad, refl, upsample)
        if ctx.has_bias and ctx.needs_input_grad[2]:
            db = torch.empty(Cout, dtype=_F32, device=x.device)
            _channel_sum(g, db, N, Cout, g.shape[2] * g.shape[3])
        return dx, dw_, db, None, None, None, None, None


_UP_A = ((0., 0., 1.), (0., 1., 1.), (1., 1., 0.), (1., 0., 0.))


_UP_MAT = {}


def _up_matrix(device):
    m = _UP_MAT.get(device)
    if m is None:
        m = _UP_MAT[device] = torch.tensor(_UP_A, dtype=_F32, device=device)
    return m


def _derived(w, tag, compose):
    cache = None
    if getattr(w, "_og_epoch", None) is not None or not w.requires_grad:
        try:
            cache = w.__dict__.setdefault("_og_derived", {})
        except AttributeError:
            pass
    if cache is None:
        return compose(w.detach()).contiguous(), False
    stamp = (w._version, _epoch_of(w), w.data_ptr())
    ent = cache.get(tag)
    if ent is not None and ent[0] == stamp:
        return ent[1], True
    val = compose(w.detach())
    out = ent[1] if (ent is not None and ent[0][2] == stamp[2]) else torch.empty(val.shape, dtype=_F32, device=w.device)
    out.copy_(val)
    cache[tag] = (stamp, out)
    return out, True


def _up_bank(w):
    def compose(wd):
        A = _up_matrix(wd.device)
        return torch.einsum("pk,mckl,ql->cmpq", A, wd, A)
    return _derived(w, "up4", compose)


def _up_phased_ok(x, w, bias, stride, pad, pad_mode, upsample, act):
    return (upsample and stride == 1 and pad == 1 and pad_mode != "reflect" and bias is None
            and act in (None, "none") and w.shape[2] == 3 and w.shape[3] == 3 and w.shape[0] > 32
            and x.shape[1] > 32 and x.shape[2] >= 2 and x.shape[3] >= 2 and _MATH["mode"] != 1
            and float(x.shape[0]) * max(x.shape[1], 4 * w.shape[0]) * x.shape[2] * x.shape[3] * 4.0 < 4.0e9)


class _UpConv3x3Fn(torch.autograd.Function):
    @staticmethod
    def forward(ctx, x, w):
        _chk(x, w)
        x = _c(x)
        w = _c(w)
        N, C, H, W = x.shape
        M = w.shape[0]
        if w.shape[1] != C:
            raise _lib.ObjganHipError("conv2d: bad weight shape %s for input %s" % (tuple(w.shape), tuple(x.shape)))
        W4, cacheable = _up_bank(w)
        y = _conv_dgrad(x, W4, N, M, 2 * H, 2 * W, 2, 1, 0, False, cacheable)
        ctx.save_for_backward(x, w)
        return y

    @staticmethod
    def backward(ctx, dy):
        x, w = ctx.saved_tensors
        dy = _c(dy)
        _chk(dy)
        C, M = x.shape[1], w.shape[0]
        dx = dw_ = None
        if ctx.needs_input_grad[0]:
            W4, _ = _up_bank(w)
            dx = _conv_fwd(dy, W4, None, 2, 1, 0, False, None)
        if ctx.needs_input_grad[1]:
            dW4 = _conv_wgrad(dy, x, C, 4, 2, 1, 0, False)
            A = _up_matrix(x.device)
            dw_ = torch.einsum("pk,cmpq,ql->mckl", A, dW4, A).contiguous()
        return dx, dw_


def _w_slice(w, lo, hi):
    return _derived(w, (lo, hi), lambda wd: wd[:, lo:hi])


class _Conv2dCatFn(torch.autograd.Function):

    @staticmethod
    def forward(ctx, x1, x2, w, stride, pad, act):
        _chk(x1, x2, w)
        x = torch.cat([x1, x2], dim=1)
        w = _c(w)
        if w.shape[1] != x.shape[1] or w.shape[2] != w.shape[3]:
            raise _lib.ObjganHipError("conv2d_cat: bad weight shape %s for inputs %s + %s"
                                      % (tuple(w.shape), tuple(x1.shape), tuple(x2.shape)))
        y = _conv_fwd(x, w, None, stride, pad, 0, False, act)
        ctx.cfg = (stride, pad, act, w.shape[2], x1.shape[1])
        ctx.save_for_backward(x, w, y if act not in (None, "none") else None)
        return y

    @staticmethod
    def backward(ctx, dy):
        x, w, y = ctx.saved_tensors
        stride, pad, act, k, c1 = ctx.cfg
        N, C, H, W = x.shape
        dy = _c(dy)
        _chk(dy)
        g = _act_grad(dy, y, act)
        n1, n2, nw = ctx.needs_input_grad[0], ctx.needs_input_grad[1], ctx.needs_input_grad[2]
        dx1 = dx2 = dw_ = None
        if n1 and n2:
            dx = _conv_dgrad(g, w, N, C, H, W, stride, pad, 0, False)
            dx1, dx2 = dx[:, :c1], dx[:, c1:]
        elif n1:
            ws, ok = _w_slice(w, 0, c1)
            dx1 = _conv_dgrad(g, ws, N, c1, H, W, stride, pad, 0, False, cacheable=ok)
        elif n2:
            ws, ok = _w_slice(w, c1, C)
            dx2 = _conv_dgrad(g, ws, N, C - c1, H, W, stride, pad, 0, False, cacheable=ok)
        if nw:
            dw_ = _conv_wgrad(x, g, w.shape[0], k, stride, pad, 0, False, sink=_grad_sink(w, tuple(w.shape)))
        return dx1, dx2, dw_, None, None, None


def conv2d_cat(x1, x2, w, stride=1, pad=0, act=None):
    return _Conv2dCatFn.apply(x1, x2, w, stride, pad, act)


def conv2d(x, w, bias=None, stride=1, pad=0, pad_mode="zeros", upsample=False, act=None):
    if _up_phased_ok(x, w, bias, stride, pad, pad_mode, upsample, act):
        return _UpConv3x3Fn.apply(x, w)
    return _Conv2dFn.apply(x, w, bias, stride, pad, pad_mode, upsample, act)


class _ConvFrozenFn(torch.autograd.Function):

    @staticmethod
    def forward(ctx, x, w, bias, stride, ph, pw, act):
        _chk(x, w, bias)
        if w.requires_grad or (bias is not None and bias.requires_grad):
            raise _lib.ObjganHipError("conv2d_frozen: the filter bank must not require gradients")
        x, w = _c(x), _c(w)
        y = _conv_fwd(x, w, bias, stride, (ph, pw), 0, False, act)
        ctx.cfg = (stride, ph, pw, act, tuple(x.shape))
        ctx.save_for_backward(w, y if act not in (None, "none") else None)
        return y

    @staticmethod
    def backward(ctx, dy):
        w, y = ctx.saved_tensors
        stride, ph, pw, act, (N, Cin, H, W) = ctx.cfg
        if not ctx.needs_input_grad[0]:
            return None, None, None, None, None, None, None
        g = _act_grad(_c(dy), y, act)
        return _conv_dgrad(g, w, N, Cin, H, W, stride, (ph, pw), 0, False), None, None, None, None, None, None


def conv2d_frozen(x, w, bias=None, stride=1, pad=(0, 0), act=None):
    return _ConvFrozenFn.apply(x, w, bias, int(stride), int(pad[0]), int(pad[1]), act)


def linear(x, w, bias=None, act=None):
    w4 = w.reshape(w.shape[0], w.shape[1], 1, 1)
    cell = getattr(w, "_og_epoch", None)
    if cell is not None and w4 is not w:
        w4._og_epoch = cell
    y = conv2d(x.reshape(x.shape[0], x.shape[1], 1, 1), w4, bias, 1, 0, "zeros", False, act)
    return y.reshape(x.shape[0], w.shape[0])


_NORM_MODE = {None: 0, "none": 0, "lrelu": 1, "glu": 2}


_LAST_AMAX = [None]


class _NormActFn(torch.autograd.Function):
    @staticmethod
    def forward(ctx, x, gamma, beta, residual, running_mean, running_var, per_channel, mode, eps,
                momentum):
        _chk(x, gamma, beta, residual, running_mean, running_var)
        x = _c(x)
        N, C = x.shape[0], x.shape[1]
        HW = x.numel() // (N * C) if x.numel() else 0
        Co = C // 2 if mode == "glu" else C
        y = torch.empty((N, Co) + tuple(x.shape[2:]), dtype=_F32, device=x.device)
        G = C if per_channel else N * C
        nst = _q("objgan_norm_ws_floats", N, C, HW, int(per_channel))
        ws = torch.empty(nst + 2 * G, dtype=_F32, device=x.device)
        sums, mean, rstd = ws[:nst], ws[nst:nst + G], ws[nst + G:]
        residual = _c(residual) if residual is not None else None
        emit = _q("objgan_norm_amax_supported", N, C, HW, int(per_channel), int(gamma is not None)) \
            if _amax_wanted(y.numel()) else 0
        am = (_amax_zeroed(x.device) if emit == 2 else torch.empty(_AMAX_SLOTS, dtype=_F32, device=x.device)) if emit else None
        _lib.call("objgan_norm_forward", _p(x), _p(y), _p(residual), _p(gamma), _p(beta),
                  _p(running_mean), _p(running_var), _p(sums), _p(mean), _p(rstd),
                  N, C, HW, int(per_channel), _NORM_MODE[mode], float(eps), float(momentum), _p(am), _stream())
        _LAST_AMAX[0] = am
        ctx.cfg = (N, C, HW, int(per_channel), _NORM_MODE[mode], emit)
        ctx.has_res = residual is not None
        ctx.save_for_backward(x, mean, rstd, gamma, beta)
        return y

    @staticmethod
    def backward(ctx, dy):
        x, mean, rstd, gamma, beta = ctx.saved_tensors
        N, C, HW, per_channel, mode, emit = ctx.cfg
        dy = _c(dy)
        _chk(dy)
        G = C if per_channel else N * C
        bsums = torch.empty(_q("objgan_norm_ws_floats", N, C, HW, int(per_channel)), dtype=_F32, device=x.device)
        dx = torch.empty_like(x)
        dgamma = dbeta = None
        if gamma is not None:
            dgamma = torch.empty_like(gamma)
            dbeta = torch.empty_like(beta)
        am = ((_amax_zeroed(x.device) if emit == 2 else torch.empty(_AMAX_SLOTS, dtype=_F32, device=x.device))
              if (emit and _amax_wanted(dx.numel())) else None)
        _lib.call("objgan_norm_backward", _p(x), _p(dy), _p(mean), _p(rstd), _p(gamma), _p(beta),
                  _p(bsums), _p(dx), _p(dgamma), _p(dbeta), N, C, HW, per_channel, mode, _p(am), _stream())
        if am is not None:
            _amax_attach(dx, am)
        dres = dy if ctx.has_res else None
        return dx, dgamma, dbeta, dres, None, None, None, None, None, None


def norm_act(x, gamma=None, beta=None, residual=None, running_mean=None, running_var=None,
             per_channel=False, mode=None, eps=1e-5, momentum=0.1):
    _LAST_AMAX[0] = None
    y = _NormActFn.apply(x, gamma, beta, residual, running_mean, running_var, per_channel, mode,
                         eps, momentum)
    if _LAST_AMAX[0] is not None:
        _amax_attach(y, _LAST_AMAX[0])
        _LAST_AMAX[0] = None
    return y


def norm_act_eval(x, gamma, beta, running_mean, running_var, mode=None, eps=1e-5):
    _chk(x, gamma, beta, running_mean, running_var)
    if x.requires_grad and torch.is_grad_enabled():
        raise _lib.ObjganHipError("eval-mode BatchNorm is forward-only: wrap the call in torch.no_grad()")
    x = _c(x)
    N, C = x.shape[0], x.shape[1]
    HW = x.numel() // (N * C) if x.numel() else 0
    Co = C // 2 if mode == "glu" else C
    y = torch.empty((N, Co) + tuple(x.shape[2:]), dtype=_F32, device=x.device)
    rstd = torch.rsqrt(running_var + eps)
    _lib.call("objgan_norm_apply", _p(x), _p(y), None, _p(gamma), _p(beta), _p(running_mean), _p(rstd),
              N, C, HW, 1, _NORM_MODE[mode], _stream())
    return y


def _mask_u8(mask):
    if mask is None:
        return None
    if not mask.is_cuda:
        raise _lib.ObjganHipError("attention mask must live on the GPU")
    return _c(mask.to(torch.uint8))


class _AttnGeneralFn(torch.autograd.Function):

    @staticmethod
    def forward(ctx, x, src, mask_u8):
        _chk(x, src)
        x = _c(x)
        src = _c(src)
        B, idf = x.shape[0], x.shape[1]
        Q = x.shape[2] * x.shape[3]
        L = src.shape[2]
        wc = torch.empty_like(x)
        attn = torch.empty((B, L, x.shape[2], x.shape[3]), dtype=_F32, device=x.device)
        _lib.call("objgan_attn_general_forward", _p(x), _p(src), _p(mask_u8), _p(wc), _p(attn),
                  B, idf, Q, L, _stream())
        ctx.save_for_backward(x, src, attn)
        return wc, attn

    @staticmethod
    def backward(ctx, dwc, dattn):
        x, src, attn = ctx.saved_tensors
        B, idf = x.shape[0], x.shape[1]
        Q = x.shape[2] * x.shape[3]
        L = src.shape[2]
        dwc = _c(dwc)
        dattn = _c(dattn) if dattn is not None else None
        dx = torch.empty_like(x)
        dsrc = torch.empty_like(src)
        ws = torch.empty(_lib.load().objgan_attn_general_backward_ws_floats(B, idf, Q, L), dtype=_F32, device=x.device)
        _lib.call("objgan_attn_general_backward", _p(x), _p(src), _p(attn), _p(dwc), _p(dattn),
                  _p(dx), _p(dsrc), B, idf, Q, L, _p(ws), _stream())
        return dx, dsrc, None


def attn_general(x, src, mask=None):
    return _AttnGeneralFn.apply(x, src, _mask_u8(mask))


class _AttnBUFn(torch.autograd.Function):

    @staticmethod
    def forward(ctx, tgt, ctx1, src, mask_u8, normalize, eps):
        _chk(tgt, ctx1, src)
        if tgt.requires_grad or ctx1.requires_grad:
            raise _lib.ObjganHipError(
                "attn_bu: gradients w.r.t. the label / GloVe features are not implemented "
                "(they are constants on the training hot path)")
        tgt, ctx1, src = _c(tgt), _c(ctx1), _c(src)
        B, d2, R = tgt.shape[0], tgt.shape[1], tgt.shape[2] * tgt.shape[3]
        idf, L = src.shape[1], src.shape[2]
        wc = torch.empty((B, idf, tgt.shape[2], tgt.shape[3]), dtype=_F32, device=tgt.device)
        attn = torch.empty((B, L, tgt.shape[2], tgt.shape[3]), dtype=_F32, device=tgt.device)
        _lib.call("objgan_attn_bu_forward", _p(tgt), _p(ctx1), _p(src), _p(mask_u8), _p(wc), _p(attn),
                  B, d2, idf, R, L, int(normalize), float(eps), _stream())
        ctx.save_for_backward(attn)
        ctx.dims = (B, idf, R, L)
        ctx.mark_non_differentiable(attn)
        return wc, attn

    @staticmethod
    def backward(ctx, dwc, dattn):
        (attn,) = ctx.saved_tensors
        B, idf, R, L = ctx.dims
        dwc = _c(dwc)
        dsrc = torch.empty((B, idf, L), dtype=_F32, device=dwc.device)
        _lib.call("objgan_attn_bu_backward", _p(dwc), _p(attn), _p(dsrc), B, idf, R, L, _stream())
        return None, None, dsrc, None, None, None


def attn_bu(tgt, ctx1, src, mask=None, normalize=True, eps=1e-8):
    return _AttnBUFn.apply(tgt, ctx1, src, _mask_u8(mask), normalize, eps)


class _MaskedMaxFn(torch.autograd.Function):

    @staticmethod
    def forward(ctx, f, m, ih, iw):
        _chk(f, m)
        B, num, R = f.shape[0], f.shape[1], f.shape[2]
        f2 = _c(f.reshape(B, num, R))
        P = ih * iw
        if m.dim() == 4:
            if not (m.stride(3) == 1 and m.stride(2) == iw):
                m = _c(m)
            sb, sr, sc = m.stride(0), m.stride(1), 0
        elif m.dim() == 5:
            if m.stride(2) == 0 and m.stride(4) == 1 and m.stride(3) == iw:
                sb, sr, sc = m.stride(0), m.stride(1), 0
            else:
                m = _c(m)
                sb, sr, sc = R * num * P, num * P, P
        else:
            raise _lib.ObjganHipError("masked_max: mask must be 4-D or 5-D")
        out = torch.empty((B, num, ih, iw), dtype=_F32, device=f.device)
        _lib.call("objgan_masked_max_forward", _p(f2), _p(m), _p(out), B, num, R, P, sb, sr, sc, _stream())
        ctx.save_for_backward(f2, m)
        ctx.geom = (B, num, R, P, sb, sr, sc, tuple(f.shape))
        return out

    @staticmethod
    def backward(ctx, dout):
        f2, m = ctx.saved_tensors
        B, num, R, P, sb, sr, sc, fshape = ctx.geom
        dout = _c(dout)
        df = torch.empty((B, num, R), dtype=_F32, device=f2.device)
        ws = torch.empty(_lib.load().objgan_masked_max_backward_ws_floats(B, num, R, P), dtype=_F32, device=f2.device)
        _lib.call("objgan_masked_max_backward", _p(f2), _p(m), _p(dout), _p(df), B, num, R, P,
                  sb, sr, sc, _p(ws), _stream())
        return df.reshape(fshape), None, None, None


def masked_max(f, m, ih, iw):
    return _MaskedMaxFn.apply(f, m, ih, iw)


def _bmm_raw(A, B):
    Bt, M, K = A.shape
    N = B.shape[2]
    C = torch.empty((Bt, M, N), dtype=_F32, device=A.device)
    _lib.call("objgan_bmm_strided", _p(A), _p(B), _p(C), Bt, M, N, K,
              A.stride(0), A.stride(1), A.stride(2), B.stride(0), B.stride(1), B.stride(2),
              C.stride(0), C.stride(1), C.stride(2), _stream())
    return C


class _BmmFn(torch.autograd.Function):
    @staticmethod
    def forward(ctx, A, B):
        _chk(A, B)
        if A.dim() != 3 or B.dim() != 3 or A.shape[0] != B.shape[0] or A.shape[2] != B.shape[1]:
            raise _lib.ObjganHipError("bmm: shapes %s x %s" % (tuple(A.shape), tuple(B.shape)))
        ctx.save_for_backward(A, B)
        return _bmm_raw(A, B)

    @staticmethod
    def backward(ctx, dC):
        A, B = ctx.saved_tensors
        _chk(dC)
        dA = _bmm_raw(dC, B.transpose(1, 2)) if ctx.needs_input_grad[0] else None
        dB = _bmm_raw(A.transpose(1, 2), dC) if ctx.needs_input_grad[1] else None
        return dA, dB


def bmm(A, B):
    return _BmmFn.apply(A, B)


class _BceConstFn(torch.autograd.Function):
    @staticmethod
    def forward(ctx, prob, target):
        _chk(prob)
        prob = _c(prob)
        out = torch.empty((), dtype=_F32, device=prob.device)
        _lib.call("objgan_bce_const_forward", _p(prob), _p(out), prob.numel(), float(target), _stream())
        ctx.save_for_backward(prob)
        ctx.target = float(target)
        return out

    @staticmethod
    def backward(ctx, g):
        (prob,) = ctx.saved_tensors
        g = _c(g)
        _chk(g)
        dp = torch.empty_like(prob)
        _lib.call("objgan_bce_const_backward", _p(prob), _p(g), _p(dp), prob.numel(), ctx.target, _stream())
        return dp, None


def bce_const(prob, target):
    return _BceConstFn.apply(prob, target)


class _SoftmaxStridedFn(torch.autograd.Function):
    @staticmethod
    def forward(ctx, x, dim, scale, lens, rowvalid):
        _chk(x)
        x = _c(x)
        d = dim % x.dim()
        outer = int(math.prod(x.shape[:d]))
        n = x.shape[d]
        inner = int(math.prod(x.shape[d + 1:]))
        y = torch.empty_like(x)
        _lib.call("objgan_softmax_strided_forward", _p(x), _p(y), outer, n, inner, float(scale),
                  _p(lens), 0 if lens is None else lens.numel(), _p(rowvalid), _stream())
        ctx.save_for_backward(y)
        ctx.geom = (outer, n, inner, float(scale))
        return y

    @staticmethod
    def backward(ctx, dy):
        (y,) = ctx.saved_tensors
        outer, n, inner, scale = ctx.geom
        dy = _c(dy)
        dx = torch.empty_like(y)
        _lib.call("objgan_softmax_strided_backward", _p(y), _p(dy), _p(dx), outer, n, inner, scale, _stream())
        return dx, None, None, None, None


def softmax_strided(x, dim, scale=1.0, lens=None, rowvalid=None):
    return _SoftmaxStridedFn.apply(x, dim, scale, lens, rowvalid)


class RoIAlignFunction(torch.autograd.Function):

    @staticmethod
    def forward(ctx, features, rois, aligned_height, aligned_width, spatial_scale):
        _chk(features, rois)
        features = _c(features)
        rois = _c(rois)
        B, C, H, W = features.shape
        num_rois = rois.shape[0]
        roi_cols = rois.shape[1] if rois.dim() == 2 else 0
        out = torch.zeros((num_rois, C, aligned_height, aligned_width), dtype=_F32, device=features.device)
        _lib.call("objgan_roi_align_forward", _p(features), _p(rois), _p(out), num_rois, roi_cols,
                  C, H, W, aligned_height, aligned_width, float(spatial_scale), _stream())
        ctx.save_for_backward(rois)
        ctx.geom = (B, C, H, W, aligned_height, aligned_width, float(spatial_scale))
        return out

    @staticmethod
    def backward(ctx, grad_output):
        (rois,) = ctx.saved_tensors
        B, C, H, W, ah, aw, scale = ctx.geom
        grad_output = _c(grad_output)
        _chk(grad_output)
        grad_input = torch.zeros((B, C, H, W), dtype=_F32, device=grad_output.device)
        need = _lib.load().objgan_roi_align_backward_ws_floats(B, rois.shape[0], C, H, W, ah, aw)
        ws = torch.empty((max(int(need), 1),), dtype=_F32, device=grad_output.device)
        _lib.call("objgan_roi_align_backward_ordered", _p(grad_output), _p(rois), _p(grad_input), B,
                  rois.shape[0], rois.shape[1], C, H, W, ah, aw, scale, _p(ws), int(need), _stream())
        return grad_input, None, None, None, None


def roi_align(features, rois, aligned_height, aligned_width, spatial_scale):
    return RoIAlignFunction.apply(features, rois, int(aligned_height), int(aligned_width), float(spatial_scale))


class _AvgPool2s1Fn(torch.autograd.Function):
    @staticmethod
    def forward(ctx, x):
        _chk(x)
        x = _c(x)
        ih, iw = x.shape[-2], x.shape[-1]
        planes = x.numel() // (ih * iw) if x.numel() else 0
        y = torch.empty(tuple(x.shape[:-2]) + (ih - 1, iw - 1), dtype=_F32, device=x.device)
        _lib.call("objgan_avgpool2s1_forward", _p(x), _p(y), planes, ih, iw, _stream())
        ctx.geom = (tuple(x.shape), planes, ih, iw)
        return y

    @staticmethod
    def backward(ctx, dy):
        shape, planes, ih, iw = ctx.geom
        dy = _c(dy)
        dx = torch.empty(shape, dtype=_F32, device=dy.device)
        _lib.call("objgan_avgpool2s1_backward", _p(dy), _p(dx), planes, ih, iw, _stream())
        return dx


def avgpool2s1(x):
    return _AvgPool2s1Fn.apply(x)


class _Pool2dFn(torch.autograd.Function):

    @staticmethod
    def forward(ctx, x, k, s, p, mode):
        _chk(x)
# ... 224 lines not shown
        if a.shape[2] != 3:
            raise _lib.ObjganHipError("images_to_device: host-decoded images must be uint8 [H, W, 3], got %s" % (a.shape,))
        host.numpy()[o:o + a.size] = a.reshape(-1)
        offs[i], hs[i], ws[i] = total + o, a.shape[0], a.shape[1]
        o += (a.size + 15) // 16 * 16
    parts.append(host.to(device, non_blocking=True))
    return torch.cat(parts), np.asarray(offs, np.int64), hs, ws


def jpeg_decode(files, device, cache=None, keys=None):
    out, offs, hs, ws = jpeg_decode_batch(files, device, cache, keys)
    return [out[int(o):int(o) + h * w * 3].view(h, w, 3) for o, h, w in zip(offs, hs, ws)]


def resize_pil_bilinear_device(src, offs, hs, ws, sizes):
    import numpy as np
    device = src.device
    B = len(hs)
    hs_d = torch.tensor(list(hs), dtype=torch.int32).to(device)
    ws_d = torch.tensor(list(ws), dtype=torch.int32).to(device)
    offs_d = torch.from_numpy(np.asarray(offs, np.int64)).to(device)
    Hmax = max(hs)
    side = max(max(hs), max(ws))
    outs = []
    for S in sizes:
        S = int(S)
        kmax = int(_lib.load().objgan_resize_pil_kmax(side, S))
        coef = torch.empty(B * 2 * S * (kmax + 2), dtype=torch.int32, device=device)
        tmp = torch.empty(B * Hmax * S * 3, dtype=torch.uint8, device=device)
        out = torch.empty((B, 3, S, S), dtype=_F32, device=device)
        _lib.call("objgan_resize_pil_rgb8", _p(src), _p(offs_d), _p(hs_d), _p(ws_d), B, Hmax, kmax, S,
                  _p(coef), _p(tmp), _p(out), _stream())
        outs.append(out)
    return outs


def resize_pil_bilinear(images, sizes, device):
    import numpy as np
    arrs = [np.ascontiguousarray(im.numpy() if torch.is_tensor(im) else im, dtype=np.uint8) for im in images]
    for a in arrs:
        if a.ndim != 3 or a.shape[2] != 3 or a.shape[0] < 1 or a.shape[1] < 1:
            raise _lib.ObjganHipError("resize_pil_bilinear: images must be uint8 [H, W, 3], got %s" % (a.shape,))
    device = torch.device(device)
    if device.type != "cuda":
        raise _lib.ObjganHipError("resize_pil_bilinear: needs a HIP device (no CPU path)")
    B = len(arrs)
    sizes_b = [a.size for a in arrs]
    offs = np.concatenate(([0], np.cumsum(sizes_b)[:-1])).astype(np.int64) if B else np.zeros(0, np.int64)
    host = torch.empty(int(sum(sizes_b)), dtype=torch.uint8).pin_memory()
    flat = host.numpy()
    for a, o in zip(arrs, offs):
        flat[o:o + a.size] = a.reshape(-1)
    src = host.to(device, non_blocking=True)
    hs = torch.tensor([a.shape[0] for a in arrs], dtype=torch.int32).to(device)
    ws = torch.tensor([a.shape[1] for a in arrs], dtype=torch.int32).to(device)
    offs_d = torch.from_numpy(offs).to(device)
    Hmax = max(a.shape[0] for a in arrs)
    side = max(max(a.shape[0], a.shape[1]) for a in arrs)
    outs = []
    for S in sizes:
        S = int(S)
        kmax = int(_lib.load().objgan_resize_pil_kmax(side, S))
        coef = torch.empty(B * 2 * S * (kmax + 2), dtype=torch.int32, device=device)
        tmp = torch.empty(B * Hmax * S * 3, dtype=torch.uint8, device=device)
        out = torch.empty((B, 3, S, S), dtype=_F32, device=device)
        _lib.call("objgan_resize_pil_rgb8", _p(src), _p(offs_d), _p(hs), _p(ws), B, Hmax, kmax, S,
                  _p(coef), _p(tmp), _p(out), _stream())
        outs.append(out)
    return outs


def _gaussian_taps(sigma, truncate=4.0):
    import numpy as np
    radius = int(truncate * float(sigma) + 0.5)
    x = np.arange(-radius, radius + 1)
    phi = np.exp(-0.5 / (sigma * sigma) * x ** 2)
    return phi / phi.sum()


def resize_masks(masks, sizes):
    if not masks.is_cuda or masks.dtype != torch.float64 or masks.dim() < 2 or masks.shape[-1] != masks.shape[-2]:
        raise _lib.ObjganHipError("resize_masks: float64 [..., n, n] on the GPU (got %s %s on %s; no CPU path)"
                                  % (masks.dtype, tuple(masks.shape), masks.device))
    n = int(masks.shape[-1])
    sizes = [int(S) for S in sizes]
    if not 2 <= n <= 64 or not 1 <= len(sizes) <= 4:
        raise _lib.ObjganHipError("resize_masks: n <= 64 and at most four sizes")
    src = _c(masks)
    lead = tuple(src.shape[:-2])
    count = 1
    for d in lead:
        count *= int(d)
    outs = [torch.empty(lead + (S, S), dtype=torch.float64, device=src.device) for S in sizes]
    ntaps, taps = [], [0.0] * (17 * len(sizes))
    for k, S in enumerate(sizes):
        if S < n:
            w = _gaussian_taps((n / float(S) - 1.0) / 2.0)
            if len(w) > 17:
                raise _lib.ObjganHipError("resize_masks: shrinking %d -> %d is outside the table (radius <= 8)" % (n, S))
            ntaps.append(len(w))
            taps[17 * k:17 * k + len(w)] = [float(v) for v in w]
        else:
            ntaps.append(0)
    outp = (ctypes.c_void_p * len(sizes))(*[o.data_ptr() for o in outs])
    _lib.call("objgan_mask_resize", _p(src), count, n, len(sizes), _iarr(sizes), outp, _iarr(ntaps),
              (ctypes.c_double * len(taps))(*taps), _stream())
    return outs


_EXPAND = {}


def expansion_matrix(a, vis, sigma=20.0):
    import numpy as np
    a, vis = int(a), int(vis)

    def mirror(i, n):
        if n == 1:
            return 0
        i = i % (2 * n - 2)
        return i if i < n else 2 * n - 2 - i

    Z = np.zeros((vis, a), np.float64)
    for o in range(vis):
        c = (o + 0.5) * (a / float(vis)) - 0.5
        if a == 1:
            c = 0.0
        elif c < 0:
            c = -c
        i = int(np.floor(c))
        f = c - i
        Z[o, mirror(i, a)] += 1.0 - f
        Z[o, mirror(i + 1, a)] += f
    w = _gaussian_taps(sigma)
    r = len(w) // 2
    G = np.zeros((vis, vis), np.float64)
    for o in range(vis):
        for k in range(-r, r + 1):
            G[o, mirror(o + k, vis)] += w[k + r]
    return G.dot(Z)


def _expansion_matrix_dev(a, vis, device):
    key = (int(a), int(vis), str(device))
    m = _EXPAND.get(key)
    if m is None:
        m = _EXPAND[key] = torch.from_numpy(expansion_matrix(a, vis)).pin_memory().to(device, non_blocking=True)
    return m


def paste_blend_table():
    import numpy as np
    table = np.empty((256, 256), np.uint8)
    _lib.call("objgan_snapshot_blend_table", ctypes.c_void_p(table.ctypes.data))
    return table


SNAPSHOT_NORMS = {"global": 0, "panel": 1, "raw": 2, "panel_unguarded": 3}


def snapshot_grid(imgs, attn_maps, att_sze, text_strip, lr_imgs=None, max_word_num=12, font_max=50, nvis=8,
                  per_panel_norm=None, norm=None):
    if norm is None:
        norm = "panel" if per_panel_norm else "global"
    elif per_panel_norm is not None:
        raise _lib.ObjganHipError("snapshot_grid: give norm= or per_panel_norm=, not both")
    if norm not in SNAPSHOT_NORMS:
        raise _lib.ObjganHipError("snapshot_grid: norm is one of %s (got %r)" % (sorted(SNAPSHOT_NORMS), norm))
    as_list = isinstance(attn_maps, (list, tuple))
    _chk(imgs, lr_imgs, *(attn_maps if as_list else (attn_maps,)))
    if not (torch.is_tensor(text_strip) and text_strip.is_cuda and text_strip.dtype == torch.uint8):
        raise _lib.ObjganHipError("snapshot_grid: text_strip is a uint8 tensor on the GPU (there is no CPU path)")
    if imgs.dim() != 4 or imgs.shape[1] != 3 or (lr_imgs is not None and (lr_imgs.dim() != 4 or lr_imgs.shape[1] != 3)):
        raise _lib.ObjganHipError("snapshot_grid: images are [B, 3, h, w]")
    B, a, nvis, font_max, mw = int(imgs.shape[0]), int(att_sze), int(nvis), int(font_max), int(max_word_num)
    H, W = int(imgs.shape[2]), int(imgs.shape[3])
    vis = a * 16 if a == 17 else H
    if (not 1 <= nvis <= B or (len(attn_maps) if as_list else attn_maps.shape[0]) < nvis
            or (lr_imgs is not None and lr_imgs.shape[0] < nvis)):
        raise _lib.ObjganHipError("snapshot_grid: nvis = %d images wanted, batch of %d" % (nvis, B))
    counts = None
    if as_list:
        per = [m.detach().reshape(-1, a, a) for m in attn_maps[:nvis]]
        sizes = [int(m.shape[0]) for m in per]
        attn = torch.zeros((nvis, max(sizes + [1]), a, a), dtype=_F32, device=imgs.device)
        for i, m in enumerate(per):
            attn[i, :sizes[i]].copy_(m)
        if min(sizes) < 1:
            raise _lib.ObjganHipError("snapshot_grid: an image without attention maps")
        counts = torch.tensor(sizes, dtype=torch.int32).pin_memory().to(imgs.device, non_blocking=True)
    else:
        attn = _c(attn_maps.detach()).reshape(int(attn_maps.shape[0]), -1, a, a)
    T = int(attn.shape[1])
    ratio = vis // a
    if ratio < 1 or (ratio == 1 and vis != a) or not 1 <= T <= 1023:
        raise _lib.ObjganHipError("snapshot_grid: %d maps of %d x %d cannot be drawn into %d x %d panels" % (T, a, a, vis, vis))
    width = (mw + 2) * (vis + 2)
    if tuple(text_strip.shape) != (nvis * font_max, width, 3):
        raise _lib.ObjganHipError("snapshot_grid: text_strip is %s, expected %s"
                                  % (tuple(text_strip.shape), (nvis * font_max, width, 3)))
    imgs = _c(imgs.detach())
    lr = _c(lr_imgs.detach()) if lr_imgs is not None else None
    LH, LW = (int(lr.shape[2]), int(lr.shape[3])) if lr is not None else (0, 0)
    if ratio > 1 and SNAPSHOT_NORMS[norm] >= 2:
        raise _lib.ObjganHipError("snapshot_grid: norm=%r draws maps at their own size (maps %d x %d, panels %d x %d)"
                                  % (norm, a, a, vis, vis))
    M = _expansion_matrix_dev(a, vis, imgs.device) if ratio > 1 else None
    nws = _q("objgan_snapshot_ws_doubles", nvis, T, a, vis)
    ws = torch.empty(nws, dtype=torch.float64, device=imgs.device)
    out = torch.empty((nvis * (font_max + 2 * vis), width, 3), dtype=torch.uint8, device=imgs.device)
    _lib.call("objgan_snapshot_grid", _p(imgs), _p(lr), _p(attn), _p(counts), _p(M), _p(_c(text_strip)), _p(out), _p(ws), nws,
              nvis, T, a, vis, H, W, LH, LW, mw, font_max, SNAPSHOT_NORMS[norm], _stream())
    return out


def mask_to_rgb8(masks, sel=None):
    _chk(masks)
    if masks.dim() < 2:
        raise _lib.ObjganHipError("mask_to_rgb8: masks are [..., h, w]")
    h, w = int(masks.shape[-2]), int(masks.shape[-1])
    planes = masks.numel() // max(h * w, 1)
    if h * w < 1 or planes < 1:
        raise _lib.ObjganHipError("mask_to_rgb8: no pixels in masks of shape %s" % (tuple(masks.shape),))
    m = _c(masks.detach())
    sel_dev, N = None, planes
    if sel is not None:
        if torch.is_tensor(sel) and sel.is_cuda:
            lo, hi, N = int(sel.min()), int(sel.max()), int(sel.numel())
            sel_dev = _c(sel.to(torch.int32).reshape(-1))
        else:
            import numpy as np
            host = np.asarray(sel.numpy() if torch.is_tensor(sel) else sel, dtype=np.int64).reshape(-1)
            N = int(host.size)
            if N < 1:
                raise _lib.ObjganHipError("mask_to_rgb8: empty selection")
            lo, hi = int(host.min()), int(host.max())
            sel_dev = torch.from_numpy(host.astype(np.int32)).pin_memory().to(m.device, non_blocking=True)
        if lo < 0 or hi >= planes:
            raise _lib.ObjganHipError("mask_to_rgb8: selection %d .. %d outside the %d planes" % (lo, hi, planes))
    out = torch.empty((N, h, w, 3), dtype=torch.uint8, device=m.device)
    _lib.call("objgan_mask_to_rgb8", _p(m), _p(sel_dev), _p(out), N, h * w, _stream())
    return out


_LIFT_TABLES = {}


def _lift_axis_tables(n_in, n_out, device):
    key = (n_in, n_out, str(device))
    ent = _LIFT_TABLES.get(key)
    if ent is not None:
        return ent
    import numpy as np
    scale = np.float32(n_in - 1) / np.float32(n_out - 1) if n_out > 1 else np.float32(0)
    i0s, i1s, l1s, offs, idxs, wts = [], [], [], [], [], []
    base = 0
    for d in (-1, 0, 1):
        r = np.arange(n_out, dtype=np.int64) + d
        r = np.where(r < 0, -r, r)
        r = np.where(r >= n_out, 2 * (n_out - 1) - r, r)
        src = (scale * r.astype(np.float32)).astype(np.float32)
        i0 = np.minimum(src.astype(np.int32), n_in - 1)
        i1 = i0 + (i0 < n_in - 1)
        l1 = (src - i0.astype(np.float32)).astype(np.float32)
        l0 = (np.float32(1.0) - l1).astype(np.float32)
        i0s.append(i0); i1s.append(i1); l1s.append(l1)
        q = np.concatenate([i0, i1]).astype(np.int64)
        o = np.concatenate([np.arange(n_out), np.arange(n_out)])
        wv = np.concatenate([l0, l1])
        order = np.lexsort((o, q))
        q, o, wv = q[order], o[order], wv[order]
        off = np.zeros(n_in + 1, np.int64)
        np.add.at(off, q + 1, 1)
        off = np.cumsum(off) + base
        base = int(off[-1])
        offs.append(off); idxs.append(o); wts.append(wv)
    def t(arrays, dt, flat=False):
        a = np.concatenate(arrays) if flat else np.stack(arrays)
        return torch.from_numpy(np.ascontiguousarray(a.astype(dt))).to(device)
    longest = max(int((o[1:] - o[:-1]).max()) for o in offs)
    if longest > 8:
        raise _lib.ObjganHipError("lift_stem_conv: lift factor %d -> %d too large for the adjoint kernel" % (n_in, n_out))
    ent = (t(i0s, np.int32), t(i1s, np.int32), t(l1s, np.float32),
           t(offs, np.int32), t(idxs, np.int32, True), t(wts, np.float32, True))
    _LIFT_TABLES[key] = ent
    return ent


class _LiftTapsFn(torch.autograd.Function):
    @staticmethod
    def forward(ctx, z, bias, SH, SW):
        _chk(z, bias)
        z = _c(z)
        N, C9, h, w = z.shape
        Mo = C9 // 9
        rows = _lift_axis_tables(h, SH, z.device)
        cols = _lift_axis_tables(w, SW, z.device)
        y = torch.empty((N, Mo, SH, SW), dtype=_F32, device=z.device)
        scratch = torch.empty(N * 3 * Mo * h * SW, dtype=_F32, device=z.device)
        _lib.call("objgan_lift_taps_forward", _p(z), _p(bias), _p(y), _p(scratch), N, Mo, h, w, SH, SW,
                  _p(cols[0]), _p(cols[1]), _p(cols[2]), _p(rows[0]), _p(rows[1]), _p(rows[2]), _stream())
        ctx.geom = (N, Mo, h, w, SH, SW)
        ctx.has_bias = bias is not None
        return y

    @staticmethod
    def backward(ctx, dy):
        N, Mo, h, w, SH, SW = ctx.geom
        dy = _c(dy)
        _chk(dy)
        dz = db = None
        if ctx.needs_input_grad[0]:
            rows = _lift_axis_tables(h, SH, dy.device)
            cols = _lift_axis_tables(w, SW, dy.device)
            dz = torch.empty((N, 9 * Mo, h, w), dtype=_F32, device=dy.device)
            scratch = torch.empty(N * 3 * Mo * h * SW, dtype=_F32, device=dy.device)
            _lib.call("objgan_lift_taps_backward", _p(dy), _p(dz), _p(scratch), N, Mo, h, w, SH, SW,
                      _p(rows[3]), _p(rows[4]), _p(rows[5]), _p(cols[3]), _p(cols[4]), _p(cols[5]), _stream())
        if ctx.has_bias and ctx.needs_input_grad[1]:
            db = torch.empty(Mo, dtype=_F32, device=dy.device)
            _channel_sum(dy, db, N, Mo, SH * SW)
        return dz, db, None, None


def lift_stem_conv(seg, w, bias, size):
    Mo, C = w.shape[0], w.shape[1]
    if w.shape[2] != 3 or w.shape[3] != 3:
        raise _lib.ObjganHipError("lift_stem_conv: 3x3 filter bank expected")
    w9 = w.permute(2, 3, 0, 1).reshape(9 * Mo, C, 1, 1).contiguous()
    w9._og_nocache = True
    z = conv2d(seg, w9)
    return _LiftTapsFn.apply(z, bias, int(size), int(size))


def lstm_bidir_forward(table, captions, lens, wt_ih, wt_hh, b_ih, b_hh, max_len, return_cn=False):
    _chk(table, wt_ih, wt_hh, b_ih, b_hh)
    if not captions.is_cuda or captions.dtype != torch.int64:
        raise _lib.ObjganHipError("lstm: captions must be an int64 tensor on the GPU")
    captions = _c(captions)
    lens = _c(lens.to(device=captions.device, dtype=torch.int32))
    B, L = captions.shape
    I, G = wt_ih.shape[1], wt_ih.shape[2]
    H = G // 4
    out = torch.empty((B, 2 * H, int(max_len)), dtype=_F32, device=captions.device)
    hn = torch.empty((B, 2 * H), dtype=_F32, device=captions.device)
    if return_cn:
        cn = torch.empty((B, 2 * H), dtype=_F32, device=captions.device)
        _lib.call("objgan_lstm_bidir_forward_state", _p(table), _p(captions), _p(lens), _p(wt_ih), _p(wt_hh),
                  _p(b_ih), _p(b_hh), _p(out), _p(hn), _p(cn), B, L, int(max_len), I, H, table.shape[0], _stream())
        return out, hn, cn
    _lib.call("objgan_lstm_bidir_forward", _p(table), _p(captions), _p(lens), _p(wt_ih), _p(wt_hh),
              _p(b_ih), _p(b_hh), _p(out), _p(hn), B, L, int(max_len), I, H, table.shape[0], _stream())
    return out, hn


def box_decode_cpw():
    return int(_lib.load().objgan_box_decode_default_cpw())


def box_decode(h0, c0, noise, weights, first_input, sos, eos, trace=False, cpw=None):
    _chk(h0, c0, *weights)
    if not noise.is_cuda or noise.dtype != torch.float64 or noise.dim() != 3 or noise.shape[2] != 6:
        raise _lib.ObjganHipError("box_decode: noise must be a [B, T, 6] float64 tensor on the GPU")
    if len(weights) != 17:
        raise _lib.ObjganHipError("box_decode: 17 weight tensors expected")
    h0, c0, noise = _c(h0), _c(c0), _c(noise)
    weights = [_c(w) for w in weights]
    B, H = h0.shape
    T = noise.shape[1]
    l_emb, xy_w, wt_ih, wt_hh, lo_wt, xyo_wt, who_wt = (weights[i] for i in (0, 1, 7, 8, 11, 13, 15))
    L, A, K = l_emb.shape[0], xy_w.shape[0], xyo_wt.shape[1] // 6
    shapes = [(L, H), (A, 2), (A,), (A, 2), (A,), (A, 2), (A,), (2 * A + H, 4 * H), (H, 4 * H), (4 * H,), (4 * H,),
              (H, L), (L,), (H + L, 6 * K), (6 * K,), (H + L + A, 6 * K), (6 * K,)]
    if tuple(c0.shape) != (B, H) or noise.shape[0] != B or [tuple(w.shape) for w in weights] != shapes:
        raise _lib.ObjganHipError("box_decode: inconsistent shapes")
    dev = h0.device
    labels = torch.empty((B, T), dtype=torch.int32, device=dev)
    lengths = torch.empty((B,), dtype=torch.int32, device=dev)
    samples = torch.empty((B, T, 4), dtype=torch.float64, device=dev)
    tr = torch.empty((B, T, L + 12 * K), dtype=_F32, device=dev) if trace else None
    x0, y0, w0, r0 = (float(v) for v in first_input)
    _lib.call("objgan_box_decode", _p(h0), _p(c0), _p(noise), *[_p(w) for w in weights], x0, y0, w0, r0,
              _p(labels), _p(lengths), _p(samples), _p(tr), B, T, H, L, K, A, int(sos), int(eos),
              box_decode_cpw() if cpw is None else int(cpw), _stream())
    return (labels, lengths, samples, tr) if trace else (labels, lengths, samples)


def box_weight_shapes(H, L, K, A):
    return [(L, H), (A, 2), (A,), (A, 2), (A,), (A, 2), (A,), (2 * A + H, 4 * H), (H, 4 * H), (4 * H,), (4 * H,),
            (H, L), (L,), (H + L, 6 * K), (6 * K,), (H + L + A, 6 * K), (6 * K,)]


def box_arena(shapes, device, fill=None):
    sizes = [int(math.prod(s)) for s in shapes]
    flat = torch.zeros(sum(sizes), dtype=_F32, device=device)
    views, o = [], 0
    for s, n in zip(shapes, sizes):
        views.append(flat[o:o + n].view(s))
        o += n
    if fill is not None:
        for v, t in zip(views, fill):
            v.copy_(t)
    return flat, views


def _box_train_dims(weights, name):
    if len(weights) != 17:
        raise _lib.ObjganHipError("%s: 17 weight tensors expected" % name)
    L, H = weights[0].shape
    A, K = weights[1].shape[0], weights[13].shape[1] // 6
    if [tuple(w.shape) for w in weights] != box_weight_shapes(H, L, K, A) or any(not w.is_contiguous() for w in weights):
        raise _lib.ObjganHipError("%s: the 17 tensors must be contiguous, in the kernel's layout" % name)
    return H, L, K, A


def _box_targets(labels, boxes, lens, B, name):
    for t, dt in ((labels, torch.int32), (boxes, _F32), (lens, torch.int32)):
        if not t.is_cuda:
            raise _lib.ObjganHipError("%s: targets must be on the GPU (got a %s tensor); there is no CPU path"
                                      % (name, t.device))
        if t.dtype != dt or not t.is_contiguous():
            raise _lib.ObjganHipError("%s: labels / lens are contiguous int32, boxes contiguous fp32" % name)
    if labels.dim() != 2 or labels.shape[0] != B or labels.shape[1] < 2 or \
            tuple(boxes.shape) != (B, labels.shape[1], 4) or tuple(lens.shape) != (B,):
        raise _lib.ObjganHipError("%s: labels [B, T + 1], boxes [B, T + 1, 4], lens [B] expected" % name)
    return labels.shape[1] - 1


def box_train_ws_floats(B, T, H, L, K, A):
    n = int(_lib.load().objgan_box_train_ws_floats(B, T, H, L, K, A))
    if n <= 0 and B > 0:
        raise _lib.ObjganHipError("box_train: shape outside the kernel's limits")
    return n


def box_train_forward(h0, c0, labels, boxes, lens, weights, first_input, ws=None, cpw=None):
    _chk(h0, c0, *weights)
    H, L, K, A = _box_train_dims(weights, "box_train_forward")
    h0, c0 = _c(h0), _c(c0)
    B = h0.shape[0]
    if tuple(h0.shape) != (B, H) or tuple(c0.shape) != (B, H):
        raise _lib.ObjganHipError("box_train_forward: h0, c0 must be [B, H]")
    T = _box_targets(labels, boxes, lens, B, "box_train_forward")
    need = box_train_ws_floats(B, T, H, L, K, A)
    if ws is None:
        ws = torch.empty(max(need, 1), dtype=_F32, device=h0.device)
    _chk(ws)
    trace = torch.empty((B, T, L + 12 * K), dtype=_F32, device=h0.device)
    x0, y0, w0, r0 = (float(v) for v in first_input)
    _lib.call("objgan_box_train_forward", _p(h0), _p(c0), _p(labels), _p(boxes), _p(lens), *[_p(w) for w in weights],
              x0, y0, w0, r0, _p(trace), _p(ws), ws.numel(), B, T, H, L, K, A,
              box_decode_cpw() if cpw is None else int(cpw), _stream())
    return trace, ws


def box_train_loss(trace, labels, boxes, lens, weight, lamda1, lamda2, K, pad=0):
    _chk(trace, weight)
    trace, weight = _c(trace), _c(weight)
    B = trace.shape[0]
    T = _box_targets(labels, boxes, lens, B, "box_train_loss")
    L = weight.numel()
    if trace.dim() != 3 or trace.shape[1] != T or trace.shape[2] != L + 12 * K:
        raise _lib.ObjganHipError("box_train_loss: trace must be [B, T, L + 12K]")
    sums = torch.zeros(4 * B + 1, dtype=torch.float64, device=trace.device)
    dtrace = torch.empty_like(trace)
    _lib.call("objgan_box_train_loss", _p(trace), _p(labels), _p(boxes), _p(lens), _p(weight), float(lamda1),
              float(lamda2), _p(sums), _p(dtrace), B, T, L, int(K), int(pad), _stream())
    return sums, dtrace


def box_train_backward(dtrace, trace, c0, labels, lens, weights, ws, grads=None, cpw=None):
    _chk(dtrace, trace, c0, ws, *weights)
    H, L, K, A = _box_train_dims(weights, "box_train_backward")
    dtrace, trace, c0 = _c(dtrace), _c(trace), _c(c0)
    B, T = trace.shape[0], trace.shape[1]
    if tuple(dtrace.shape) != tuple(trace.shape) or trace.shape[2] != L + 12 * K or tuple(c0.shape) != (B, H) or \
            tuple(labels.shape) != (B, T + 1) or labels.dtype != torch.int32 or not labels.is_cuda or \
            tuple(lens.shape) != (B,) or lens.dtype != torch.int32 or not lens.is_cuda:
        raise _lib.ObjganHipError("box_train_backward: inconsistent shapes")
    if grads is None:
        grads = box_arena(box_weight_shapes(H, L, K, A), trace.device)[1]
    _chk(*grads)
    if [tuple(g.shape) for g in grads] != box_weight_shapes(H, L, K, A) or any(not g.is_contiguous() for g in grads):
        raise _lib.ObjganHipError("box_train_backward: 17 contiguous gradient tensors in the kernel's layout expected")
    ptrs = (ctypes.c_void_p * 17)(*[g.data_ptr() for g in grads])
    _lib.call("objgan_box_train_backward", _p(dtrace), _p(trace), _p(c0), _p(_c(labels)), _p(_c(lens)),
              _p(weights[7]), _p(weights[8]), _p(weights[11]), _p(weights[13]), _p(weights[15]), ptrs, _p(ws),
              ws.numel(), B, T, H, L, K, A, box_decode_cpw() if cpw is None else int(cpw), _stream())
    return grads


def box_train_clip(flat_grads, max_norm, partials=None, out=None):
    _chk(flat_grads, out)
    if partials is None:
        partials = torch.empty(256, dtype=torch.float64, device=flat_grads.device)
    if out is None:
        out = torch.empty(2, dtype=_F32, device=flat_grads.device)
    if not partials.is_cuda or partials.dtype != torch.float64 or partials.numel() < 256 or out.numel() < 2:
        raise _lib.ObjganHipError("box_train_clip: partials is >= 256 float64, out 2 floats, on the GPU")
    _lib.call("objgan_box_train_clip", _p(_c(flat_grads)), flat_grads.numel(), float(max_norm), _p(partials), _p(out),
              _stream())
    return out


def adam_step_(p, g, m, v, lr, beta1, beta2, eps, step, grad_scale=1.0, n=None):
    _chk(p, g, m, v)
    n = p.numel() if n is None else int(n)
    _lib.call("objgan_adam_step", _p(p), _p(g), _p(m), _p(v), n, float(lr), float(beta1),
              float(beta2), float(eps), int(step), float(grad_scale), _stream())


def adam_step_gated_(p, g, m, v, lr, beta1, beta2, eps, state, flag, coef, grad_scale=1.0, n=None):
    _chk(p, g, m, v, flag, coef)
    if not state.is_cuda or state.dtype != torch.float64 or state.numel() < 3:
        raise _lib.ObjganHipError("adam_step_gated_: state must be 3 float64 values on the GPU")
    n = p.numel() if n is None else int(n)
    _lib.call("objgan_adam_step_gated", _p(p), _p(g), _p(m), _p(v), n, float(lr), float(beta1),
              float(beta2), float(eps), _p(state), _p(flag), _p(coef), float(grad_scale), _stream())


def ema_update_(avg, p, decay):
    _chk(avg, p)
    _lib.call("objgan_ema_update", _p(avg), _p(p), p.numel(), float(decay), float(1.0 - decay), _stream())


def _off(t, floats):
    return ctypes.c_void_p(t.data_ptr() + 4 * int(floats))


def _gate_slices(w, Cin):
    wx, okx = _w_slice(w, 0, Cin)
    wh, okh = _w_slice(w, Cin, w.shape[1])
    for s, ok in ((wx, okx), (wh, okh)):
        if not ok:
            s._og_nocache = True
    return wx, okx, wh, okh


def convlstm_cell_forward_(gx, gx_bstride, gh, c_prev, h_out, h_slab, slab_bstride, c_out, acts, B, Ch, HW):
    _chk(gh, c_prev, h_out, c_out, acts)
    _lib.call("objgan_convlstm_cell_forward", gx, _p(gh), _p(c_prev), _p(h_out), h_slab, _p(c_out), _p(acts),
              int(B), int(Ch), int(HW), int(gx_bstride), int(slab_bstride), _stream())


def convlstm_cell_backward_(dh_slab, dh_bstride, dh_rec, dc_in, acts, c_prev, dg_slab, dg_bstride, dg_out, dc_out, B, Ch, HW):
    _chk(dh_rec, dc_in, acts, c_prev, dg_out, dc_out)
    _lib.call("objgan_convlstm_cell_backward", dh_slab, _p(dh_rec), _p(dc_in), _p(acts), _p(c_prev), dg_slab, _p(dg_out),
              _p(dc_out), int(B), int(Ch), int(HW), int(dh_bstride), int(dg_bstride), _stream())


class _ConvLstmSeqFn(torch.autograd.Function):

    @staticmethod
    def forward(ctx, x, w, bias, reverse):
        _chk(x, w, bias)
        x = _c(x)
        B, R, Cin, H, W = x.shape
        Ch = w.shape[0] // 4
        k = w.shape[2]
        if w.shape[0] != 4 * Ch or w.shape[1] != Cin + Ch or k != w.shape[3] or k % 2 != 1 or R > 255:
            raise _lib.ObjganHipError("convlstm_sequence: bad gate bank %s for input %s" % (tuple(w.shape), tuple(x.shape)))
        pad = k // 2
        HW = H * W
        wx, okx, wh, okh = _gate_slices(w, Cin)
        dev = x.device
        x2 = x.view(B * R, Cin, H, W)
        gx = _conv_fwd(x2, wx, bias, 1, pad, 0, False, None)
        hs = torch.empty((R, B, Ch, H, W), dtype=_F32, device=dev)
        cs = torch.empty((R, B, Ch, H, W), dtype=_F32, device=dev)
        acts = torch.empty((R, B, 5 * Ch, H, W), dtype=_F32, device=dev)
        slab = torch.empty((B, R, Ch, H, W), dtype=_F32, device=dev)
        for t in range(R):
            gh = _conv_fwd(hs[t - 1], wh, None, 1, pad, 0, False, None) if t else None
            slot = R - 1 - t if reverse else t
            convlstm_cell_forward_(_off(gx, t * 4 * Ch * HW), R * 4 * Ch * HW, gh, cs[t - 1] if t else None, hs[t],
                                   _off(slab, slot * Ch * HW), R * Ch * HW, cs[t], acts[t], B, Ch, HW)
        ctx.cfg = (bool(reverse), pad, k, okx, okh)
        ctx.has_bias = bias is not None
        ctx.save_for_backward(x2, w, hs, cs, acts)
        return slab

    @staticmethod
    def backward(ctx, dslab):
        x2, w, hs, cs, acts = ctx.saved_tensors
        reverse, pad, k, _, _ = ctx.cfg
        R, B, Ch, H, W = hs.shape
        Cin = x2.shape[1]
        HW = H * W
        dslab = _c(dslab)
        _chk(dslab)
        dev = dslab.device
        wx, okx, wh, okh = _gate_slices(w, Cin)
        dgs = torch.empty((B, R, 4 * Ch, H, W), dtype=_F32, device=dev)
        dgt = torch.empty((R, B, 4 * Ch, H, W), dtype=_F32, device=dev)
        dh_rec = dc = None
        for t in range(R - 1, -1, -1):
            slot = R - 1 - t if reverse else t
            dc_new = torch.empty((B, Ch, H, W), dtype=_F32, device=dev)
            convlstm_cell_backward_(_off(dslab, slot * Ch * HW), R * Ch * HW, dh_rec, dc, acts[t], cs[t - 1] if t else None,
                                    _off(dgs, t * 4 * Ch * HW), R * 4 * Ch * HW, dgt[t], dc_new, B, Ch, HW)
            dc = dc_new
            if t:
                dh_rec = _conv_dgrad(dgt[t], wh, B, Ch, H, W, 1, pad, 0, False, cacheable=okh)
        dg2 = dgs.view(B * R, 4 * Ch, H, W)
        dx = dw_ = db = None
        if ctx.needs_input_grad[0]:
            dx = _conv_dgrad(dg2, wx, B * R, Cin, H, W, 1, pad, 0, False, cacheable=okx).view(B, R, Cin, H, W)
        if ctx.needs_input_grad[1]:
            dwx = _conv_wgrad(x2, dg2, 4 * Ch, k, 1, pad, 0, False)
            if R > 1:
                dwh = _conv_wgrad(hs[:R - 1].view((R - 1) * B, Ch, H, W), dgt[1:].view((R - 1) * B, 4 * Ch, H, W),
                                  4 * Ch, k, 1, pad, 0, False)
            else:
                dwh = torch.zeros((4 * Ch, Ch, k, k), dtype=_F32, device=dev)
            dw_ = torch.cat([dwx, dwh], dim=1)
        if ctx.has_bias and ctx.needs_input_grad[2]:
            db = torch.empty(4 * Ch, dtype=_F32, device=dev)
            _channel_sum(dg2, db, B * R, 4 * Ch, HW)
        return dx, dw_, db, None


def convlstm_sequence(x, w, bias=None, reverse=False):
    return _ConvLstmSeqFn.apply(x, w, bias, bool(reverse))

# ... 244 lines not shown
```

Baseline: 123.0 images/sec.

## Fuse small-group norm stats/apply into single kernels and accumulate param grads in place

Adds single-block-per-group forward and backward norm kernels for shapes that need no split reduction. Each fuses the statistics reduction, finalize and apply steps, replacing separate stats, finalize and apply launches. Norm affine and bias gradient paths can now accumulate straight into the parameter's grad buffer through a grad sink, avoiding separate temporaries and the autograd accumulation add. This reduces launch count and small-tensor traffic, but it gives up parallelism for groups that were previously spread across more blocks, and it depends on the grad-sink semantics being correct.

```diff
diff --git a/include/objgan_hip.h b/include/objgan_hip.h
--- a/include/objgan_hip.h
+++ b/include/objgan_hip.h
@@ -121,9 +121,15 @@
                          const float* gamma, const float* beta, float* bsums,
                          float* dx, float* dgamma, float* dbeta,
                          int N, int C, int HW, int per_channel, int mode, float* amax, void* stream);
+int objgan_norm_backward_acc(const float* x, const float* dy, const float* mean, const float* rstd,
+                             const float* gamma, const float* beta, float* bsums,
+                             float* dx, float* dgamma, float* dbeta,
+                             int N, int C, int HW, int per_channel, int mode, float* amax, int accumulate, void* stream);
+int objgan_norm_set_fold(int on);
 int objgan_act_backward(const float* dy, const float* y, float* dz, long total, int kind, float* amax, void* stream);
 long objgan_channel_sum_ws_floats(int N, int C, int HW);
 int objgan_channel_sum(const float* x, float* out, int N, int C, int HW, float* ws, void* stream);
+int objgan_channel_sum_acc(const float* x, float* out, int N, int C, int HW, float* ws, int accumulate, void* stream);
 
 int objgan_attn_general_forward(const float* x, const float* src, const unsigned char* mask,
                                 float* wc, float* attn, int B, int idf, int Q, int L, void* stream);
diff --git a/obj-gan_amd/csrc/norm.hip b/obj-gan_amd/csrc/norm.hip
--- a/obj-gan_amd/csrc/norm.hip
+++ b/obj-gan_amd/csrc/norm.hip
@@ -28,10 +28,8 @@
     ws.sums[2 * g] = a; ws.sums[2 * g + 1] = b;
 }
 
-__global__ __launch_bounds__(256) void norm_stats_kernel(const float* __restrict__ x,
-                                                         NormWs ws, NormGeom gm) {
-    __shared__ float red[16];
-    const int g = blockIdx.x;
+__device__ __forceinline__ void og_stats_slice(const float* __restrict__ x, const NormGeom& gm, int g, float* red,
+                                               float& s1_out, float& s2_out) {
     const int planes = gm.per_channel ? gm.N : 1;
     const size_t base = gm.per_channel ? (size_t)g * gm.HW : (size_t)g * gm.HW;
     const size_t pstride = (size_t)gm.C * gm.HW;
@@ -48,9 +46,33 @@
         s1 += d;
         s2 += d * d;
     }
-    s1 = og_block_sum(s1, red);
-    s2 = og_block_sum(s2, red);
+    s1_out = og_block_sum(s1, red);
+    s2_out = og_block_sum(s2, red);
+}
+
+__global__ __launch_bounds__(256) void norm_stats_kernel(const float* __restrict__ x,
+                                                         NormWs ws, NormGeom gm) {
+    __shared__ float red[16];
+    const int g = blockIdx.x;
+    float s1, s2;
+    og_stats_slice(x, gm, g, red, s1, s2);
     if (threadIdx.x == 0) og_store_partial2(ws, g, blockIdx.y, s1, s2);
+}
+
+__device__ __forceinline__ void og_stats_from_sums(float K, float s1, float s2, float cnt, float eps,
+                                                   float& mu, float& rs, float& var_out) {
+    const float m1 = s1 / cnt;
+    float var = s2 / cnt - m1 * m1;
+    var = fmaxf(var, 0.f);
+    mu = K + m1;
+    rs = 1.0f / sqrtf(var + eps);
+    var_out = var;
+}
+__device__ __forceinline__ void og_running_update(float* __restrict__ running_mean, float* __restrict__ running_var, int g,
+                                                  float mu, float var, float cnt, float momentum) {
+    const float unbiased = cnt > 1.f ? var * cnt / (cnt - 1.f) : var;
+    running_mean[g] = (1.f - momentum) * running_mean[g] + momentum * mu;
+    running_var[g] = (1.f - momentum) * running_var[g] + momentum * unbiased;
 }
 
 __global__ __launch_bounds__(256) void norm_finalize_kernel(
@@ -61,17 +83,28 @@
     if (g >= G) return;
     const float cnt = gm.per_channel ? (float)gm.N * gm.HW : (float)gm.HW;
     const float K = x[(size_t)g * gm.HW];
-    const float m1 = sums[2 * g] / cnt;
-    float var = sums[2 * g + 1] / cnt - m1 * m1;
-    var = fmaxf(var, 0.f);
-    const float mu = K + m1;
+    float mu, rs, var;
+    og_stats_from_sums(K, sums[2 * g], sums[2 * g + 1], cnt, eps, mu, rs, var);
     mean[g] = mu;
-    rstd[g] = 1.0f / sqrtf(var + eps);
-    if (running_mean) {
-        const float unbiased = cnt > 1.f ? var * cnt / (cnt - 1.f) : var;
-        running_mean[g] = (1.f - momentum) * running_mean[g] + momentum * mu;
-        running_var[g] = (1.f - momentum) * running_var[g] + momentum * unbiased;
-    }
+    rstd[g] = rs;
+    if (running_mean) og_running_update(running_mean, running_var, g, mu, var, cnt, momentum);
+}
+
+__device__ __forceinline__ float og_norm_z(float x, float mu, float rs, const float* __restrict__ gamma,
+                                           const float* __restrict__ beta, int c) {
+#pragma clang fp contract(off)
+    const float z = (x - mu) * rs;
+    return gamma ? fmaf(z, gamma[c], beta[c]) : z;
+}
+__device__ __forceinline__ float og_norm_act(float za, float zb, int mode) {
+#pragma clang fp contract(off)
+    if (mode == OG_NORM_GLU) return za * og_sigmoid(zb);
+    if (mode == OG_NORM_LRELU) return za > 0.f ? za : 0.2f * za;
+    return za;
+}
+__device__ __forceinline__ float og_add_residual(float v, float r) {
+#pragma clang fp contract(off)
+    return v + r;
 }
 
 __global__ __launch_bounds__(256) void norm_apply_kernel(
@@ -88,21 +121,15 @@
         const int c = (int)(plane - (long)n * Co);
         const int ga = gm.per_channel ? c : n * gm.C + c;
         const size_t xa = ((size_t)n * gm.C + c) * gm.HW + i;
-        float za = (x[xa] - mean[ga]) * rstd[ga];
-        if (gamma) za = za * gamma[c] + beta[c];
-        float v;
+        const float za = og_norm_z(x[xa], mean[ga], rstd[ga], gamma, beta, c);
+        float zb = 0.f;
         if (mode == OG_NORM_GLU) {
             const int cb = c + Co;
             const int gb = gm.per_channel ? cb : n * gm.C + cb;
-            float zb = (x[xa + (size_t)Co * gm.HW] - mean[gb]) * rstd[gb];
-            if (gamma) zb = zb * gamma[cb] + beta[cb];
-            v = za * og_sigmoid(zb);
-        } else if (mode == OG_NORM_LRELU) {
-            v = za > 0.f ? za : 0.2f * za;
-        } else {
-            v = za;
-        }
-        if (residual) v += residual[e];
+            zb = og_norm_z(x[xa + (size_t)Co * gm.HW], mean[gb], rstd[gb], gamma, beta, cb);
+        }
+        float v = og_norm_act(za, zb, mode);
+        if (residual) v = og_add_residual(v, residual[e]);
         y[e] = v;
     }
 }
@@ -134,12 +161,10 @@
     return d * zp * sg * (1.f - sg);
 }
 
-__global__ __launch_bounds__(256) void norm_bwd_stats_kernel(
+__device__ __forceinline__ void og_bwd_stats_slice(
     const float* __restrict__ x, const float* __restrict__ dy, const float* __restrict__ mean,
     const float* __restrict__ rstd, const float* __restrict__ gamma, const float* __restrict__ beta,
-    NormWs ws, NormGeom gm, int mode) {
-    __shared__ float red[16];
-    const int g = blockIdx.x;
+    const NormGeom& gm, int mode, int g, float* red, float& s1_out, float& s2_out) {
     const int planes = gm.per_channel ? gm.N : 1;
     const long total = (long)planes * gm.HW;
     const long chunk = (total + gridDim.y - 1) / gridDim.y;
@@ -156,9 +181,24 @@
         s1 += dz;
         s2 += dz * xhat;
     }
-    s1 = og_block_sum(s1, red);
-    s2 = og_block_sum(s2, red);
+    s1_out = og_block_sum(s1, red);
+    s2_out = og_block_sum(s2, red);
+}
+
+__global__ __launch_bounds__(256) void norm_bwd_stats_kernel(
+    const float* __restrict__ x, const float* __restrict__ dy, const float* __restrict__ mean,
+    const float* __restrict__ rstd, const float* __restrict__ gamma, const float* __restrict__ beta,
+    NormWs ws, NormGeom gm, int mode) {
+    __shared__ float red[16];
+    const int g = blockIdx.x;
+    float s1, s2;
+    og_bwd_stats_slice(x, dy, mean, rstd, gamma, beta, gm, mode, g, red, s1, s2);
     if (threadIdx.x == 0) og_store_partial2(ws, g, blockIdx.y, s1, s2);
+}
+
+__device__ __forceinline__ float og_norm_dx(float gw, float rs, float dz, float xhat, float b0, float b1, float inv_cnt) {
+#pragma clang fp contract(off)
+    return (gw * rs) * (fmaf(-b0, inv_cnt, dz) - (xhat * b1) * inv_cnt);
 }
 
 __global__ __launch_bounds__(256) void norm_bwd_apply_kernel(
@@ -177,7 +217,89 @@
         float xhat;
         const float dz = norm_dz(x, dy, mean, rstd, gamma, beta, gm, mode, n, c, i, xhat);
         const float gw = gamma ? gamma[c] : 1.f;
-        dx[e] = gw * rstd[g] * (dz - bsums[2 * g] * inv_cnt - xhat * bsums[2 * g + 1] * inv_cnt);
+        dx[e] = og_norm_dx(gw, rstd[g], dz, xhat, bsums[2 * g], bsums[2 * g + 1], inv_cnt);
+    }
+}
+
+__global__ __launch_bounds__(256) void norm_small_fwd_kernel(
+    const float* __restrict__ x, const float* __restrict__ gamma, const float* __restrict__ beta,
+    const float* __restrict__ residual, float* __restrict__ y, float* __restrict__ mean, float* __restrict__ rstd,
+    float* __restrict__ running_mean, float* __restrict__ running_var, NormGeom gm, int mode, float eps, float momentum) {
+    __shared__ float red[16];
+    const int Co = mode == OG_NORM_GLU ? gm.C / 2 : gm.C;
+    const int n0 = gm.per_channel ? 0 : blockIdx.x / Co;
+    const int c = blockIdx.x - n0 * Co;
+    const float cnt = gm.per_channel ? (float)gm.N * gm.HW : (float)gm.HW;
+    float mu[2] = {0.f, 0.f}, rs[2] = {0.f, 0.f};
+#pragma unroll
+    for (int h = 0; h < 2; ++h) {
+        if (h == 1 && mode != OG_NORM_GLU) break;
+        const int ch = c + h * Co;
+        const int g = gm.per_channel ? ch : n0 * gm.C + ch;
+        float s1, s2, var;
+        og_stats_slice(x, gm, g, red, s1, s2);
+        og_stats_from_sums(x[(size_t)g * gm.HW], s1, s2, cnt, eps, mu[h], rs[h], var);
+        if (threadIdx.x == 0) {
+            mean[g] = mu[h];
+            rstd[g] = rs[h];
+            if (running_mean) og_running_update(running_mean, running_var, g, mu[h], var, cnt, momentum);
+        }
+    }
+    const int planes = gm.per_channel ? gm.N : 1;
+    const int total = planes * gm.HW;
+    for (int e = threadIdx.x; e < total; e += 256) {
+        const int p = e / gm.HW;
+        const int i = e - p * gm.HW;
+        const int n = gm.per_channel ? p : n0;
+        const size_t xa = ((size_t)n * gm.C + c) * gm.HW + i;
+        const size_t eo = ((size_t)n * Co + c) * gm.HW + i;
+        const float za = og_norm_z(x[xa], mu[0], rs[0], gamma, beta, c);
+        float zb = 0.f;
+        if (mode == OG_NORM_GLU) zb = og_norm_z(x[xa + (size_t)Co * gm.HW], mu[1], rs[1], gamma, beta, c + Co);
+        float v = og_norm_act(za, zb, mode);
+        if (residual) v = og_add_residual(v, residual[eo]);
+        y[eo] = v;
+    }
+}
+
+__global__ __launch_bounds__(256) void norm_small_bwd_kernel(
+    const float* __restrict__ x, const float* __restrict__ dy, const float* __restrict__ mean,
+    const float* __restrict__ rstd, const float* __restrict__ gamma, const float* __restrict__ beta,
+    float* __restrict__ dx, float* __restrict__ dgamma, float* __restrict__ dbeta, NormGeom gm, int mode, int accumulate) {
+    __shared__ float red[16];
+    const int Co = mode == OG_NORM_GLU ? gm.C / 2 : gm.C;
+    const int n0 = gm.per_channel ? 0 : blockIdx.x / Co;
+    const int c = blockIdx.x - n0 * Co;
+    const float inv_cnt = 1.0f / (gm.per_channel ? (float)gm.N * gm.HW : (float)gm.HW);
+    const int planes = gm.per_channel ? gm.N : 1;
+    const int total = planes * gm.HW;
+    float b0[2] = {0.f, 0.f}, b1[2] = {0.f, 0.f};
+#pragma unroll
+    for (int h = 0; h < 2; ++h) {
+        if (h == 1 && mode != OG_NORM_GLU) break;
+        const int ch = c + h * Co;
+        const int g = gm.per_channel ? ch : n0 * gm.C + ch;
+        og_bwd_stats_slice(x, dy, mean, rstd, gamma, beta, gm, mode, g, red, b0[h], b1[h]);
+        if (dgamma && gm.per_channel && threadIdx.x == 0) {
+            dbeta[ch] = accumulate ? dbeta[ch] + b0[h] : b0[h];
+            dgamma[ch] = accumulate ? dgamma[ch] + b1[h] : b1[h];
+        }
+    }
+#pragma unroll
+    for (int h = 0; h < 2; ++h) {
+        if (h == 1 && mode != OG_NORM_GLU) break;
+        const int ch = c + h * Co;
+        const int g = gm.per_channel ? ch : n0 * gm.C + ch;
+        const float gw = gamma ? gamma[ch] : 1.f;
+        const float rg = rstd[g];
+        for (int e = threadIdx.x; e < total; e += 256) {
+            const int p = e / gm.HW;
+            const int i = e - p * gm.HW;
+            const int n = gm.per_channel ? p : n0;
+            float xhat;
+            const float dz = norm_dz(x, dy, mean, rstd, gamma, beta, gm, mode, n, ch, i, xhat);
+            dx[((size_t)n * gm.C + ch) * gm.HW + i] = og_norm_dx(gw, rg, dz, xhat, b0[h], b1[h], inv_cnt);
+        }
     }
 }
 
@@ -353,7 +475,7 @@
     const float* __restrict__ x, const float* __restrict__ dy, const float* __restrict__ mean,
     const float* __restrict__ rstd, const float* __restrict__ gamma, const float* __restrict__ beta,
     const float* __restrict__ bsums, float* __restrict__ dx, NormGeom gm,
-    float* __restrict__ dgamma, float* __restrict__ dbeta, float* __restrict__ amax) {
+    float* __restrict__ dgamma, float* __restrict__ dbeta, float* __restrict__ amax, int accumulate) {
     __shared__ float amax_red[4];
     float vmax = 0.f;
     const int Co = MODE == OG_NORM_GLU ? gm.C / 2 : gm.C;
@@ -366,8 +488,12 @@
     const bool affine = gamma != nullptr;
     const float inv_cnt = 1.0f / (gm.per_channel ? (float)gm.N * gm.HW : (float)gm.HW);
     if (dgamma && gm.per_channel && n == 0 && blockIdx.y == 0 && threadIdx.x == 0) {
-        dbeta[c] = bsums[2 * c]; dgamma[c] = bsums[2 * c + 1];
-        if (MODE == OG_NORM_GLU) { dbeta[cb] = bsums[2 * cb]; dgamma[cb] = bsums[2 * cb + 1]; }
+        dbeta[c] = accumulate ? dbeta[c] + bsums[2 * c] : bsums[2 * c];
+        dgamma[c] = accumulate ? dgamma[c] + bsums[2 * c + 1] : bsums[2 * c + 1];
+        if (MODE == OG_NORM_GLU) {
+            dbeta[cb] = accumulate ? dbeta[cb] + bsums[2 * cb] : bsums[2 * cb];
+            dgamma[cb] = accumulate ? dgamma[cb] + bsums[2 * cb + 1] : bsums[2 * cb + 1];
+        }
     }
     const float ma = mean[ga], ra = rstd[ga];
     const float mb = MODE == OG_NORM_GLU ? mean[gb] : 0.f, rb = MODE == OG_NORM_GLU ? rstd[gb] : 0.f;
@@ -547,9 +673,12 @@
 }
 
 __global__ void norm_affine_grad_kernel(const float* __restrict__ bsums, float* __restrict__ dgamma,
-                                        float* __restrict__ dbeta, int C) {
+                                        float* __restrict__ dbeta, int C, int accumulate) {
     const int c = blockIdx.x * blockDim.x + threadIdx.x;
-    if (c < C) { dbeta[c] = bsums[2 * c]; dgamma[c] = bsums[2 * c + 1]; }
+    if (c < C) {
+        dbeta[c] = accumulate ? dbeta[c] + bsums[2 * c] : bsums[2 * c];
+        dgamma[c] = accumulate ? dgamma[c] + bsums[2 * c + 1] : bsums[2 * c + 1];
+    }
 }
 
 __device__ __forceinline__ float act_bwd_one(float d, float o, int kind) {
@@ -598,7 +727,7 @@
 
 __global__ __launch_bounds__(256) void channel_sum_kernel(const float* __restrict__ x,
                                                           float* __restrict__ out, int N, int C, int HW,
-                                                          float* __restrict__ part) {
+                                                          float* __restrict__ part, int accumulate) {
     __shared__ float red[16];
     const int c = blockIdx.x;
     const long total = (long)N * HW;
@@ -613,16 +742,16 @@
     }
     s = og_block_sum(s, red);
     if (threadIdx.x == 0) {
-        if (gridDim.y == 1) out[c] = s; else part[(size_t)c * gridDim.y + blockIdx.y] = s;
+        if (gridDim.y == 1) out[c] = accumulate ? out[c] + s : s; else part[(size_t)c * gridDim.y + blockIdx.y] = s;
     }
 }
 __global__ __launch_bounds__(256) void channel_partials_sum_kernel(const float* __restrict__ part, float* __restrict__ out,
-                                                                   int C, int S) {
+                                                                   int C, int S, int accumulate) {
     const int c = blockIdx.x * blockDim.x + threadIdx.x;
     if (c >= C) return;
     float a = 0.f;
     for (int k = 0; k < S; ++k) a += part[(size_t)c * S + k];
-    out[c] = a;
+    out[c] = accumulate ? out[c] + a : a;
 }
 
 #define OG_IN_FUSED_MAX 65536
@@ -648,7 +777,19 @@
     if (ws.P > 1) hipLaunchKernelGGL(norm_partials_sum_kernel, dim3(og_cdiv(G, 256)), dim3(256), 0, s, ws, G, amax);
 }
 
+static int g_norm_fold = 1;
+static inline bool norm_small(int N, int C, int HW, int per_channel) {
+    const int G = per_channel ? C : N * C;
+    const long per_group = per_channel ? (long)N * HW : HW;
+    return g_norm_fold && !norm_planes(N, C, HW) && norm_splits(G, per_group) == 1 && per_group < (1L << 30);
+}
+
 extern "C" {
+
+int objgan_norm_set_fold(int on) {
+    g_norm_fold = on ? 1 : 0;
+    return OG_OK;
+}
 
 int objgan_norm_amax_supported(int N, int C, int HW, int per_channel, int affine) {
     if (N <= 0 || C <= 0 || HW <= 0 || !norm_planes(N, C, HW)) return 0;
@@ -689,6 +830,11 @@
             hipLaunchKernelGGL((in_fwd_fused_kernel<OG_NORM_NONE>), grid, dim3(256), 0, s, x, residual, y, mean, rstd, gm, eps, amax);
         return og_launch_status();
     }
+    if (norm_small(N, C, HW, per_channel)) {
+        hipLaunchKernelGGL(norm_small_fwd_kernel, dim3(per_channel ? Co : N * Co), dim3(256), 0, s, x, gamma, beta, residual,
+                           y, mean, rstd, running_mean, running_var, gm, mode, eps, momentum);
+        return og_launch_status();
+    }
     const NormWs ws = norm_ws(sums, G, norm_partials(N, C, HW, per_channel));
     if (planes) {
         hipLaunchKernelGGL(norm_stats_plane_kernel, dim3(N * C, chunks), dim3(256), 0, s, x, ws, gm);
@@ -742,10 +888,10 @@
     return og_launch_status();
 }
 
-int objgan_norm_backward(const float* x, const float* dy, const float* mean, const float* rstd,
-                         const float* gamma, const float* beta, float* bsums,
-                         float* dx, float* dgamma, float* dbeta,
-                         int N, int C, int HW, int per_channel, int mode, float* amax, void* stream) {
+int objgan_norm_backward_acc(const float* x, const float* dy, const float* mean, const float* rstd,
+                             const float* gamma, const float* beta, float* bsums,
+                             float* dx, float* dgamma, float* dbeta,
+                             int N, int C, int HW, int per_channel, int mode, float* amax, int accumulate, void* stream) {
     OG_ENTRY();
     if (mode == OG_NORM_GLU && (C & 1)) return OG_BAD_ARGS;
     if (N <= 0 || C <= 0 || HW <= 0) return OG_OK;
@@ -766,6 +912,12 @@
             hipLaunchKernelGGL((in_bwd_fused_kernel<OG_NORM_NONE>), grid, dim3(256), 0, s, x, dy, mean, rstd, dx, gm, amax);
         return og_launch_status();
     }
+    if (norm_small(N, C, HW, per_channel)) {
+        const int Co = mode == OG_NORM_GLU ? C / 2 : C;
+        hipLaunchKernelGGL(norm_small_bwd_kernel, dim3(per_channel ? Co : N * Co), dim3(256), 0, s, x, dy, mean, rstd,
+                           gamma, beta, dx, dgamma, dbeta, gm, mode, accumulate);
+        return og_launch_status();
+    }
     const NormWs ws = norm_ws(bsums, G, norm_partials(N, C, HW, per_channel));
     if (planes) {
         const int Co = mode == OG_NORM_GLU ? C / 2 : C;
@@ -775,7 +927,7 @@
                            gamma, beta, ws, gm);                                                            \
         norm_sum_partials(ws, G, s, amax);                                                                  \
         hipLaunchKernelGGL((norm_bwd_apply_plane_kernel<MODE>), grid, dim3(256), 0, s, x, dy, mean, rstd,   \
-                           gamma, beta, bsums, dx, gm, dgamma, dbeta, amax);
+                           gamma, beta, bsums, dx, gm, dgamma, dbeta, amax, accumulate);
         if (mode == OG_NORM_GLU) { OG_NB(OG_NORM_GLU) } else if (mode == OG_NORM_LRELU) { OG_NB(OG_NORM_LRELU) } else { OG_NB(OG_NORM_NONE) }
 #undef OG_NB
         return og_launch_status();
@@ -790,8 +942,16 @@
     }
     if (dgamma && per_channel)
         hipLaunchKernelGGL(norm_affine_grad_kernel, dim3(og_cdiv(C, 256)), dim3(256), 0, s, bsums,
-                           dgamma, dbeta, C);
+                           dgamma, dbeta, C, accumulate);
     return og_launch_status();
+}
+
+int objgan_norm_backward(const float* x, const float* dy, const float* mean, const float* rstd,
+                         const float* gamma, const float* beta, float* bsums,
+                         float* dx, float* dgamma, float* dbeta,
+                         int N, int C, int HW, int per_channel, int mode, float* amax, void* stream) {
+    return objgan_norm_backward_acc(x, dy, mean, rstd, gamma, beta, bsums, dx, dgamma, dbeta, N, C, HW, per_channel, mode,
+                                    amax, 0, stream);
 }
 
 int objgan_act_backward(const float* dy, const float* y, float* dz, long total, int kind, float* amax,
@@ -813,16 +973,20 @@
     return S > 1 ? (long)C * S : 0;
 }
 
-int objgan_channel_sum(const float* x, float* out, int N, int C, int HW, float* ws, void* stream) {
+int objgan_channel_sum_acc(const float* x, float* out, int N, int C, int HW, float* ws, int accumulate, void* stream) {
     OG_ENTRY();
     if (N <= 0 || C <= 0 || HW <= 0) return OG_OK;
     hipStream_t s = (hipStream_t)stream;
     const int S = norm_splits(C, (long)N * HW);
     if (S > 1 && !ws) return OG_BAD_ARGS;
     dim3 grid(C, S);
-    hipLaunchKernelGGL(channel_sum_kernel, grid, dim3(256), 0, s, x, out, N, C, HW, ws);
-    if (S > 1) hipLaunchKernelGGL(channel_partials_sum_kernel, dim3(og_cdiv(C, 256)), dim3(256), 0, s, ws, out, C, S);
+    hipLaunchKernelGGL(channel_sum_kernel, grid, dim3(256), 0, s, x, out, N, C, HW, ws, accumulate);
+    if (S > 1) hipLaunchKernelGGL(channel_partials_sum_kernel, dim3(og_cdiv(C, 256)), dim3(256), 0, s, ws, out, C, S, accumulate);
     return og_launch_status();
 }
 
-}
+int objgan_channel_sum(const float* x, float* out, int N, int C, int HW, float* ws, void* stream) {
+    return objgan_channel_sum_acc(x, out, N, C, HW, ws, 0, stream);
+}
+
+}
diff --git a/obj-gan_amd/objgan_hip/_lib.py b/obj-gan_amd/objgan_hip/_lib.py
--- a/obj-gan_amd/objgan_hip/_lib.py
+++ b/obj-gan_amd/objgan_hip/_lib.py
@@ -45,8 +45,12 @@
     "objgan_norm_apply": [_ptr, _ptr, _ptr, _ptr, _ptr, _ptr, _ptr, _c_int, _c_int, _c_int, _c_int, _c_int, _ptr],
     "objgan_norm_backward": [_ptr, _ptr, _ptr, _ptr, _ptr, _ptr, _ptr, _ptr, _ptr, _ptr,
                              _c_int, _c_int, _c_int, _c_int, _c_int, _ptr, _ptr],
+    "objgan_norm_backward_acc": [_ptr, _ptr, _ptr, _ptr, _ptr, _ptr, _ptr, _ptr, _ptr, _ptr,
+                                 _c_int, _c_int, _c_int, _c_int, _c_int, _ptr, _c_int, _ptr],
+    "objgan_norm_set_fold": [_c_int],
     "objgan_act_backward": [_ptr, _ptr, _ptr, _c_long, _c_int, _ptr, _ptr],
     "objgan_channel_sum": [_ptr, _ptr, _c_int, _c_int, _c_int, _ptr, _ptr],
+    "objgan_channel_sum_acc": [_ptr, _ptr, _c_int, _c_int, _c_int, _ptr, _c_int, _ptr],
     "objgan_attn_general_forward": [_ptr, _ptr, _ptr, _ptr, _ptr, _c_int, _c_int, _c_int, _c_int, _ptr],
     "objgan_attn_general_backward": [_ptr, _ptr, _ptr, _ptr, _ptr, _ptr, _ptr, _c_int, _c_int, _c_int, _c_int, _ptr, _ptr],
     "objgan_attn_bu_forward": [_ptr, _ptr, _ptr, _ptr, _ptr, _ptr, _c_int, _c_int, _c_int, _c_int, _c_int, _c_int, _c_float, _ptr],
diff --git a/obj-gan_amd/objgan_hip/ops.py b/obj-gan_amd/objgan_hip/ops.py
--- a/obj-gan_amd/objgan_hip/ops.py
+++ b/obj-gan_amd/objgan_hip/ops.py
@@ -727,10 +727,21 @@
     return sink
 
 
-def _channel_sum(g, out, N, C, HW):
+def _channel_sum(g, out, N, C, HW, accumulate=False):
     n = _lib.load().objgan_channel_sum_ws_floats(N, C, HW)
     ws = torch.empty(n, dtype=_F32, device=g.device) if n > 0 else None
-    _lib.call("objgan_channel_sum", _p(g), _p(out), N, C, HW, _p(ws), _stream())
+    _lib.call("objgan_channel_sum_acc", _p(g), _p(out), N, C, HW, _p(ws), 1 if accumulate else 0, _stream())
+
+
+def _bias_grad(bias, g, N, C, HW):
+    sink = _grad_sink(bias, (C,)) if bias is not None else None
+    if sink is not None:
+        _channel_sum(g, sink[0], N, C, HW, accumulate=True)
+        sink[1]()
+        return None
+    db = torch.empty(C, dtype=_F32, device=g.device)
+    _channel_sum(g, db, N, C, HW)
+    return db
 
 
 def _act_grad(dy, y, act):
@@ -759,12 +770,12 @@
         y = _conv_fwd(x, w, bias, stride, pad, refl, upsample, act)
         ctx.cfg = (stride, pad, refl, bool(upsample), act, w.shape[2])
         ctx.has_bias = bias is not None
-        ctx.save_for_backward(x, w, y if act not in (None, "none") else None)
+        ctx.save_for_backward(x, w, y if act not in (None, "none") else None, bias)
         return y
 
     @staticmethod
     def backward(ctx, dy):
-        x, w, y = ctx.saved_tensors
+        x, w, y, bias = ctx.saved_tensors
         stride, pad, refl, upsample, act, k = ctx.cfg
         N, Cin, H, W = x.shape
         Cout = w.shape[0]
@@ -777,8 +788,7 @@
         if ctx.needs_input_grad[0]:
             dx = _conv_dgrad(g, w, N, Cin, H, W, stride, pad, refl, upsample)
         if ctx.has_bias and ctx.needs_input_grad[2]:
-            db = torch.empty(Cout, dtype=_F32, device=x.device)
-            _channel_sum(g, db, N, Cout, g.shape[2] * g.shape[3])
+            db = _bias_grad(bias, g, N, Cout, g.shape[2] * g.shape[3])
         return dx, dw_, db, None, None, None, None, None
 
 
@@ -954,6 +964,13 @@
 
 
 _LAST_AMAX = [None]
+
+_NORM_FOLD = {"on": True}
+
+
+def set_norm_fold(on):
+    _lib.call("objgan_norm_set_fold", 1 if on else 0)
+    _NORM_FOLD["on"] = bool(on)
 
 
 class _NormActFn(torch.autograd.Function):
@@ -993,16 +1010,29 @@
         bsums = torch.empty(_q("objgan_norm_ws_floats", N, C, HW, int(per_channel)), dtype=_F32, device=x.device)
         dx = torch.empty_like(x)
         dgamma = dbeta = None
+        sinks = None
         if gamma is not None:
-            dgamma = torch.empty_like(gamma)
-            dbeta = torch.empty_like(beta)
+            if per_channel and ctx.needs_input_grad[1] and ctx.needs_input_grad[2]:
+                sinks = (_grad_sink(gamma, gamma.shape), _grad_sink(beta, beta.shape))
+                if sinks[0] is None or sinks[1] is None:
+                    sinks = None
+            if sinks is not None:
+                dgamma, dbeta = sinks[0][0], sinks[1][0]
+            else:
+                dgamma = torch.empty_like(gamma)
+                dbeta = torch.empty_like(beta)
         am = ((_amax_zeroed(x.device) if emit == 2 else torch.empty(_AMAX_SLOTS, dtype=_F32, device=x.device))
               if (emit and _amax_wanted(dx.numel())) else None)
-        _lib.call("objgan_norm_backward", _p(x), _p(dy), _p(mean), _p(rstd), _p(gamma), _p(beta),
-                  _p(bsums), _p(dx), _p(dgamma), _p(dbeta), N, C, HW, per_channel, mode, _p(am), _stream())
+        _lib.call("objgan_norm_backward_acc", _p(x), _p(dy), _p(mean), _p(rstd), _p(gamma), _p(beta),
+                  _p(bsums), _p(dx), _p(dgamma), _p(dbeta), N, C, HW, per_channel, mode, _p(am),
+                  0 if sinks is None else 1, _stream())
         if am is not None:
             _amax_attach(dx, am)
         dres = dy if ctx.has_res else None
+        if sinks is not None:
+            sinks[0][1]()
+            sinks[1][1]()
+            dgamma = dbeta = None
         return dx, dgamma, dbeta, dres, None, None, None, None, None, None
 
 
@@ -1833,6 +1863,7 @@
                   _p(cols[0]), _p(cols[1]), _p(cols[2]), _p(rows[0]), _p(rows[1]), _p(rows[2]), _stream())
         ctx.geom = (N, Mo, h, w, SH, SW)
         ctx.has_bias = bias is not None
+        ctx.save_for_backward(bias)
         return y
 
     @staticmethod
@@ -1849,8 +1880,7 @@
             _lib.call("objgan_lift_taps_backward", _p(dy), _p(dz), _p(scratch), N, Mo, h, w, SH, SW,
                       _p(rows[3]), _p(rows[4]), _p(rows[5]), _p(cols[3]), _p(cols[4]), _p(cols[5]), _stream())
         if ctx.has_bias and ctx.needs_input_grad[1]:
-            db = torch.empty(Mo, dtype=_F32, device=dy.device)
-            _channel_sum(dy, db, N, Mo, SH * SW)
+            db = _bias_grad(ctx.saved_tensors[0], dy, N, Mo, SH * SW)
         return dz, db, None, None
 
 
```

Measured after the change: 123.3 images/sec (median of 3 runs). No clear change (+0.3%).
